# apirrone/Open_Duck_Playground

Measured on AMD Instinct MI355X. Metric: env-steps/sec open_duck_mini_v2 flat_terrain @8192 envs; 1/2/4/8-GPU scaling, higher is better.
Workload: dtype f32

## Files before the change

include/odk.h:

```cpp
#ifndef ODK_H
#define ODK_H

#include <stdint.h>

#ifdef __cplusplus
extern "C" {
#endif

typedef struct odk_model odk_model;
typedef struct odk_batch odk_batch;

enum odk_status {
  ODK_OK = 0,
  ODK_ERR_INVALID = -1,
  ODK_ERR_UNSUPPORTED = -2,
  ODK_ERR_HIP = -3,
  ODK_ERR_NOMEM = -4
};

#define ODK_NOBS 101
#define ODK_NPRIV 212
#define ODK_NOBS_STANDING 85
#define ODK_NPRIV_STANDING 153
#define ODK_ENV_JOYSTICK 0
#define ODK_ENV_STANDING 1
#define ODK_NMETRIC 8
#define ODK_NU 14

typedef struct {
  float ctrl_dt, action_scale, dof_vel_scale, max_motor_velocity;
  float noise_level, noise_gyro, noise_accelerometer, noise_gravity, noise_joint_vel;
  float qpos_noise_scale[16];
  float reward_scales[7];
  float tracking_sigma;
  float push_enable, push_interval_range[2], push_magnitude_range[2];
  float cmd_range[7][2];
  int32_t use_imitation, use_motor_speed_limits;
  int32_t autoreset;
  int32_t episode_length;
  int32_t n_substeps;
  int32_t lanes_per_env;
  int32_t env_kind;
  float reset_base_qvel;
  int32_t hfield_up_normals_only;
} odk_env_config;

typedef struct {
  float* obs_dev;
  float* priv_dev;
  float* reward_dev;
  float* done_dev;
  float* truncation_dev;
  float* metrics_dev;
} odk_outputs;

enum odk_param {
  ODK_PARAM_BODY_MASS = 0,
  ODK_PARAM_BODY_IPOS_TORSO = 1,
  ODK_PARAM_DOF_FRICTIONLOSS = 2,
  ODK_PARAM_DOF_ARMATURE = 3,
  ODK_PARAM_QPOS0 = 4,
  ODK_PARAM_KP = 5
};

const char* odk_last_error(void);
void odk_default_config(odk_env_config* cfg);
void odk_default_config_standing(odk_env_config* cfg);
void odk_obs_sizes(int env_kind, int* nobs, int* npriv);

int odk_model_load(const void* blob, uint64_t len, odk_model** out);
void odk_model_free(odk_model* m);
int odk_model_dims(const odk_model* m, int* nq, int* nv, int* nu, int* nbody);
int odk_model_obs_sizes(const odk_model* m, int env_kind, int* nobs, int* npriv);

int odk_model_reduced(const odk_model* m, int* paired, int* nvr, int* nMr, int* nHr, int* red_main, int* red_twin);
int odk_model_body_lanes(const odk_model* m, int lanes_per_env, int* out, int n);
int odk_model_env_lds_floats(const odk_model* m);

int odk_batch_create(const odk_model* m, const odk_env_config* cfg, int nenv, int device, const float* prm_table,
                     const double* dxs, int nx, const double* dys, int ny, const double* dths, int nth, const double* ranges6,
                     int nsteps_in_period, odk_batch** out);
void odk_batch_destroy(odk_batch* b);
int odk_batch_set_config(odk_batch* b, const odk_env_config* cfg);

int odk_batch_set_param(odk_batch* b, int param, const float* host_values, int count_per_env);

int odk_reset(odk_batch* b, uint32_t seed, uint32_t env_id_offset, const odk_outputs* outs, void* stream);

int odk_step(odk_batch* b, const float* action_dev, const odk_outputs* outs, void* stream);

int odk_batch_bind_commands(odk_batch* b, const float* cmd_dev, int row_stride);

#define ODK_NXTERM 12
enum odk_xterm {
  ODK_XTERM_LIN_VEL_Z = 0, ODK_XTERM_ANG_VEL_XY = 1, ODK_XTERM_ORIENTATION = 2, ODK_XTERM_BASE_HEIGHT = 3, ODK_XTERM_ENERGY = 4,
  ODK_XTERM_JOINT_POS_LIMITS = 5, ODK_XTERM_TERMINATION = 6, ODK_XTERM_POSE = 7, ODK_XTERM_FEET_SLIP = 8, ODK_XTERM_FEET_CLEARANCE = 9,
  ODK_XTERM_FEET_HEIGHT = 10, ODK_XTERM_FEET_AIR_TIME = 11
};
typedef struct {
  float scale[ODK_NXTERM];
  float base_height_target;
  float max_foot_height;
  float air_time_range[2];
  float soft_joint_pos_limit_factor;
  float pose_weight[16];
} odk_reward_terms;
int odk_batch_set_reward_terms(odk_batch* b, const odk_reward_terms* terms);
int odk_batch_bind_reward_metrics(odk_batch* b, float* dev);

int odk_batch_set_imitation_joints(odk_batch* b, const int32_t* frame_joint, int nu);

int odk_batch_set_head_joints(odk_batch* b, const int32_t* actuator, int n);

#define ODK_TRACK_NACC 12
enum { ODK_TRACK_ENDED = 0, ODK_TRACK_STEPS = 1, ODK_TRACK_SAMPLES = 2, ODK_TRACK_FALLS = 3, ODK_TRACK_REWARD = 4, ODK_TRACK_SUM = 5,
       ODK_TRACK_SQERR = 8 };
int odk_tracking_accumulate(const odk_batch* b, const float* priv_dev, const float* reward_dev, const float* done_dev,
                            const float* truncation_dev, float* acc_dev, void* stream);

int odk_batch_bind_pushes(odk_batch* b, const float* push_dev, int row_stride);

int odk_batch_bind_action_delays(odk_batch* b, const int32_t* delay_dev, int row_stride);

#define ODK_PUSH_NACC 10
enum { ODK_PUSH_PUSHED = 0, ODK_PUSH_PUSH_AT = 1, ODK_PUSH_FELL = 2, ODK_PUSH_STEPS_TO_FALL = 3, ODK_PUSH_LAST_OFF = 4, ODK_PUSH_PEAK_LIN_ERR = 5,
       ODK_PUSH_PEAK_ANG_ERR = 6, ODK_PUSH_PRE_LIN_ERR_SUM = 7, ODK_PUSH_PRE_SAMPLES = 8, ODK_PUSH_PRE_LIN_ERR_LOW = 9 };
int odk_push_accumulate(const odk_batch* b, const float* priv_dev, const float* done_dev, const float* truncation_dev,
                        const float* track_acc_dev, float lin_tol, float ang_tol, float* acc_dev, void* stream);

#define ODK_GAIT_NACC 144
#define ODK_GAIT_STRIDE 16
enum { ODK_GAIT_SAMPLES = 0, ODK_GAIT_SPEED_SUM = 1, ODK_GAIT_ABS_POWER_SUM = 2, ODK_GAIT_CONTACT = 3, ODK_GAIT_DOUBLE = 5, ODK_GAIT_FLIGHT = 6,
       ODK_GAIT_TOUCHDOWNS = 7, ODK_GAIT_SWING_STEPS_SUM = 9, ODK_GAIT_SLIP_SUM = 11, ODK_GAIT_HEIGHT_SUM = 13, ODK_GAIT_HEIGHT_SQ_SUM = 14,
       ODK_GAIT_ROLLPITCH_RATE_SQ_SUM = 15, ODK_GAIT_ACTION_RATE_SUM = 16, ODK_GAIT_PREV_CONTACT = 17, ODK_GAIT_AIR_RUN = 19,
       ODK_GAIT_TORQUE_SQ = 32, ODK_GAIT_TORQUE_PEAK = 48, ODK_GAIT_VEL_PEAK = 64, ODK_GAIT_SAT = 80, ODK_GAIT_ABS_POWER = 96,
       ODK_GAIT_RANGE_MIN = 112, ODK_GAIT_RANGE_MAX = 128 };
int odk_gait_accumulate(const odk_batch* b, const float* priv_dev, const float* done_dev, const float* truncation_dev,
                        const float* track_acc_dev, const float* torque_limit_dev , float* acc_dev ,
                        void* stream);

#define ODK_POSTURE_NACC 32
enum { ODK_POSTURE_SAMPLES = 0, ODK_POSTURE_DRIFT_SPEED_SUM = 1, ODK_POSTURE_YAW_RATE_SQ_SUM = 2, ODK_POSTURE_ROLLPITCH_RATE_SQ_SUM = 3,
       ODK_POSTURE_TILT_SUM = 4, ODK_POSTURE_TILT_PEAK = 5, ODK_POSTURE_HEIGHT_SUM = 6, ODK_POSTURE_LEG_POSE_SUM = 7, ODK_POSTURE_LEG_VEL_SUM = 8,
       ODK_POSTURE_HEAD_SQERR_SUM = 9, ODK_POSTURE_ANGLE_SUM = 16, ODK_POSTURE_ERR_SQ_SUM = 20, ODK_POSTURE_ERR_PEAK = 24,
       ODK_POSTURE_LAST_OFF = 28 };
int odk_posture_accumulate(const odk_batch* b, const float* priv_dev, const float* done_dev, const float* truncation_dev,
                           const float* track_acc_dev, float tol, float* acc_dev , void* stream);

#define ODK_IMIT_NACC 160
#define ODK_IMIT_STRIDE 16
enum { ODK_IMIT_SAMPLES = 0, ODK_IMIT_GATED = 1, ODK_IMIT_SPEED_ERR_SQ_SUM = 2, ODK_IMIT_REF_SPEED_SUM = 3, ODK_IMIT_JOINT_POS_SQ_SUM = 4,
       ODK_IMIT_JOINT_VEL_SQ_SUM = 5, ODK_IMIT_BOTH = 6, ODK_IMIT_ROBOT_ONLY = 8, ODK_IMIT_REF_ONLY = 10, ODK_IMIT_REF_TOUCHDOWNS = 12,
       ODK_IMIT_TOUCHDOWNS = 14, ODK_IMIT_LAG_SUM = 16, ODK_IMIT_LAG_ABS_SUM = 18, ODK_IMIT_PREV_CONTACT = 20, ODK_IMIT_PREV_REF = 22,
       ODK_IMIT_REF_AGE = 24,
       ODK_IMIT_POS_ERR_SUM = 32, ODK_IMIT_POS_ERR_SQ = 48, ODK_IMIT_POS_ERR_PEAK = 64, ODK_IMIT_VEL_ERR_SQ = 80, ODK_IMIT_RANGE_MIN = 96,
       ODK_IMIT_RANGE_MAX = 112, ODK_IMIT_REF_RANGE_MIN = 128, ODK_IMIT_REF_RANGE_MAX = 144 };
int odk_imitation_accumulate(const odk_batch* b, const float* priv_dev, const float* done_dev, const float* truncation_dev,
                             const float* track_acc_dev, int period_steps, float* acc_dev , void* stream);

#define ODK_SCHED_MAX_SEGMENTS 8
// ... 158 lines not shown
```

open_duck_playground_amd/csrc/odk_env_kernels.h:

```cpp
#pragma once
#include <hip/hip_runtime.h>

#include "odk_shapes.h"
#include "odk_poison.h"



template <class S> __device__ __forceinline__ const int* load_shared(float* lds, int envs, const DevModel* m) {
  int* RT = reinterpret_cast<int*>(lds + envs * EnvL<S>::TOTAL);
  {
    constexpr int T = (S::NMR + 63) / 64;
    int v[T];
#pragma unroll
    for (int t = 0; t < T; t++) { const int k = threadIdx.x + 64 * t; v[t] = m->R_ent[k < S::NMR ? k : 0]; }
#pragma unroll
    for (int t = 0; t < T; t++) { const int k = threadIdx.x + 64 * t; if (k < S::NMR) RT[k] = v[t]; }
  }
  float* SH = reinterpret_cast<float*>(RT);
  float* CT = SH + S::SH_CT;
  const int k = threadIdx.x;
  if (k < 3) { CT[k] = m->pair_mu[k]; CT[3 + k] = m->pair_invweight[k]; }
  if (k < 27) CT[6 + k] = m->pair_imp[k / 9][k % 9];
  if (k < 9) CT[33 + k] = m->plane_frame[k];
  return RT;
}

__device__ __forceinline__ float i2f(int v) { return __int_as_float(v); }
__device__ __forceinline__ int f2i(float v) { return __float_as_int(v); }
__device__ __forceinline__ float nan_to_num(float x) {
  if (isnan(x)) return 0.0f;
  if (isinf(x)) return x > 0 ? 3.4028234663852886e38f : -3.4028234663852886e38f;
  return x;
}

template <class S, int G>
__device__ __noinline__ void dump_lds(float* dbg, const float* L, int env, int lane) {
  float* o = dbg + (size_t)env * S::TOTAL;
#pragma unroll 1
  for (int k = lane; k < S::TOTAL; k += G) o[k] = L[k];
}

template <int N, int G> struct G2L {
  static constexpr int T = (N + G - 1) / G;
  float v[T];
  __device__ __forceinline__ void load(const float* __restrict__ src, int lane) {
#pragma unroll
    for (int t = 0; t < T; t++) { const int i = lane + t * G; v[t] = src[i < N ? i : 0]; }
  }
  __device__ __forceinline__ void store(float* dst, int lane) const {
#pragma unroll
    for (int t = 0; t < T; t++) { const int i = lane + t * G; if (i < N) dst[i] = v[t]; }
  }
};

template <class S, int G>
struct ParamLoad {
  float q0, mass, arm, frl, kp, ipos, dq0, darm, dfrl;
  int qadr, dadr;
  __device__ __forceinline__ void load(const DevModel* __restrict__ m, const float* __restrict__ dr, int lane) {
    static_assert(S::NQ <= G && S::NV <= G && S::NB <= G && S::NU <= G, "one parameter of each kind per lane");
    const int iq = lane < S::NQ ? lane : 0, ib = lane < S::NB ? lane : 0, iv = lane < S::NV ? lane : 0, iu = lane < S::NU ? lane : 0, i3 = lane < 3 ? lane : 0;
    q0 = m->qpos0[iq];
    mass = dr ? dr[DRL<S>::MASS + ib] : m->body_mass[ib];
    arm = m->dof_armature[iv]; frl = m->dof_frictionloss[iv];
    kp = dr ? dr[DRL<S>::KP + iu] : m->act_kp[iu];
    ipos = dr ? dr[DRL<S>::IPOS + i3] : m->body_ipos[1][i3];
    qadr = m->act_qposadr[iu]; dadr = m->act_dofadr[iu];
    dq0 = dr ? dr[DRL<S>::Q0 + iu] : 0.0f; darm = dr ? dr[DRL<S>::ARM + iu] : 0.0f; dfrl = dr ? dr[DRL<S>::FRL + iu] : 0.0f;
  }
  __device__ __forceinline__ void store(float* L, bool has_dr, int lane) const {
    if (lane < S::NQ) L[S::O_Q0 + lane] = q0;
    if (lane < S::NB) L[S::O_MASS + lane] = mass;
    if (lane < S::NV) { L[S::O_ARM + lane] = arm; L[S::O_FRL + lane] = frl; }
    if (lane < S::NU) L[S::O_KP + lane] = kp;
    if (lane < 3) L[S::O_IPOS1 + lane] = ipos;
    ODK_SYNC();
    if (has_dr && lane < S::NU) { L[S::O_Q0 + qadr] = dq0; L[S::O_ARM + dadr] = darm; L[S::O_FRL + dadr] = dfrl; }
    ODK_SYNC();
  }
};
template <class S, int G>
__device__ __forceinline__ void load_params(float* L, const DevModel* m, const float* dr, int lane) {
  ParamLoad<S, G> p;
  p.load(m, dr, lane);
  p.store(L, dr != nullptr, lane);
}

__device__ __forceinline__ int prm_nearest(const float* grid, int n, float v) {
  int best = 0;
  float bd = fabsf(grid[0] - v);
#pragma unroll
  for (int i = 1; i < 16; i++) { const float d = fabsf(grid[i] - v); if (i < n && d < bd) { bd = d; best = i; } }
  return best;
}
template <int G>
__device__ __forceinline__ void prm_eval(const DevPRM* __restrict__ p, const float* table, float dx, float dy, float dth, int i, float* out, int lane) {
  const float x = fminf(fmaxf(dx, p->ranges[0]), p->ranges[1]);
  const float y = fminf(fmaxf(dy, p->ranges[2]), p->ranges[3]);
  const float t3 = fminf(fmaxf(dth, p->ranges[4]), p->ranges[5]);
  const int ix = prm_nearest(p->dxs, p->nx, x), iy = prm_nearest(p->dys, p->ny, y), it = prm_nearest(p->dths, p->nth, t3);
  float t = (float)(i % p->nsteps) / (float)p->nsteps;
  t = fminf(fmaxf(t, 0.0f), 1.0f);
  const float* c = table + ((size_t)((ix * p->ny + iy) * p->nth + it)) * 640;
  for (int k = lane; k < 40; k += G) {
    float yv = c[k * 16];
#pragma unroll
// ... 200 lines not shown
  if (lane == 2) {
    const float yaw = -3.14f + rng_uniform(k0, kr, 0, 2) * 6.28f;
    float s, co;
    sincosf(0.5f * yaw, &s, &co);
    float q0[4] = {L[S::O_QPOS + 3], L[S::O_QPOS + 4], L[S::O_QPOS + 5], L[S::O_QPOS + 6]}, qz[4] = {co, 0, 0, s}, r[4];
    qmul(r, q0, qz);
    for (int k = 0; k < 4; k++) L[S::O_QPOS + 3 + k] = r[k];
  }
  if (lane >= 3 && lane < 9) L[S::O_QVEL + lane - 3] = -c.reset_base_qvel + rng_uniform(k0, kr, 0, 3 + NU + lane - 3) * (2.0f * c.reset_base_qvel);
  for (int u = lane; u < S::NU; u += G) {
    const float v = L[S::O_QPOS + m->act_qposadr[u]] * (0.5f + rng_uniform(k0, kr, 0, 3 + u));
    L[S::O_QPOS + m->act_qposadr[u]] = v;
    L[S::O_CTRL + u] = v;
    INFO[RL.MT + u] = c.kind != 0 ? 0.0f : m->key_ctrl[u];
  }
  if (lane < 7) {
    float v;
    sample_command(c, k0, kr, 0, 9 + NU, lane, v);
    if (a.cmd) v = a.cmd[(size_t)e * a.cmd_stride + lane];
    INFO[RL.CMD + lane] = v;
  }
  ODK_SYNC();
  forward_env<S, G, HF>(L, RT, m, a.hfield, st, lane, 1);
  if (a.dbg_lds && live) dump_lds<S, G>(a.dbg_lds, L, env, lane);
  const float pint = c.push_interval_range[0] + rng_uniform(k0, kr, 0, 17 + NU) * (c.push_interval_range[1] - c.push_interval_range[0]);
  const int push_interval_steps = (int)rintf(pint / c.ctrl_dt);
  if (c.use_imitation) prm_eval<G>(&a.prm, a.prm_table, INFO[RL.CMD], INFO[RL.CMD + 1], INFO[RL.CMD + 2], 0, L + E::O_REF, lane);
  else for (int k = lane; k < 40; k += G) L[E::O_REF + k] = 0;
  ODK_SYNC();
  float contact[2];
  foot_contact_flags(L + S::O_CDIST, contact);
  const float phase[2] = {0, 0};
  draw_block<E::NDRAW>(k0, k1, 0u, L + E::O_NZ, lane);
  build_obs<S, G>(L, m, c, contact, L + E::O_NZ, 0, phase, c.noise_level != 0.0f, lane);
  if (lane == 0) {
    INFO[RL.KEY0] = i2f((int)k0); INFO[RL.KEY1] = i2f((int)k1); INFO[RL.CTR] = i2f(1);
    INFO[RL.STEP] = i2f(0); INFO[RL.PSTEP] = i2f(0); INFO[RL.PINT] = i2f(push_interval_steps);
    INFO[RL.IMI] = i2f(0); INFO[RL.LCON] = i2f(0);
  }
  ODK_SYNC();
  if (live) {
    float* rc = a.recs + (size_t)env * R::SIZE;
    float* fs = a.first + (size_t)env * R::FSIZE;
    for (int i = lane; i < S::NQ; i += G) { rc[i] = L[S::O_QPOS + i]; fs[i] = L[S::O_QPOS + i]; }
    for (int i = lane; i < S::NV; i += G) {
      rc[S::NQ + i] = L[S::O_QVEL + i]; fs[S::NQ + i] = L[S::O_QVEL + i];
      rc[S::NQ + S::NV + i] = L[S::O_WARM + i]; fs[S::NQ + S::NV + i] = L[S::O_WARM + i];
    }
    for (int k = lane; k < R::NPRIV; k += G) {
      if (k < R::NOBS) fs[R::FOBS + k] = L[E::O_PRIV + k];
      fs[R::FOBS + R::NOBS + k] = L[E::O_PRIV + k];
    }
    for (int k = lane; k < RL.NINFO; k += G) rc[R::INFO + k] = INFO[k];
    float metrics[ODK_NMETRIC] = {0, 0, 0, 0, 0, 0, 0, 0};
    write_outputs<S, G>(a, L, env, 0.0f, 0.0f, 0.0f, metrics, lane);
    if (a.xmet && lane < ODK_NXTERM) a.xmet[(size_t)env * ODK_NXTERM + lane] = 0.0f;
  }
}

constexpr int STEP_WAVES = 2;
#ifdef ODK_PROFILE
constexpr bool STEP_DUMPS_ALWAYS = true;
#else
constexpr bool STEP_DUMPS_ALWAYS = false;
#endif
template <class S, int G, int HF, bool DBG>
__device__ __forceinline__ void step_body(const KArgs& a) {
  extern __shared__ float lds[];
  using E = EnvL<S>; using R = Rec<S>;
  constexpr int NU = S::NU;
  constexpr RecLay RL = rec_lay(NU);
  const int slot = threadIdx.x / G, lane = threadIdx.x % G;
  const int env = blockIdx.x * (64 / G) + slot;
  const bool live = env < a.nenv;
  const int e = live ? env : a.nenv - 1;
  float* L = lds + slot * E::TOTAL;
#ifdef ODK_PROFILE
  const long long t_k0 = clock64();
#endif
#ifdef ODK_POISON_LDS
  odk_poison_fill(lds, E::wg_floats(64 / G));
  ODK_SYNC();
#endif
  const int* RT = load_shared<S>(lds, 64 / G, a.m);
  const DevModel* m = a.m;
  const EnvCfg& c = a.cfg;
  float* INFO = L + E::O_INFO; float* ACT = L + E::O_ACT; float* CTRL = L + S::O_CTRL;
  float* rc = a.recs + (size_t)e * R::SIZE;
  {
    G2L<S::NQ + 2 * S::NV, G> g_state;
    G2L<RL.NINFO, G> g_info;
    G2L<NU, G> g_act;
    ParamLoad<S, G> g_par;
    const float* drp = a.dr ? a.dr + (size_t)e * DRL<S>::SIZE : nullptr;
    g_state.load(rc, lane); g_info.load(rc + R::INFO, lane); g_act.load(a.action + (size_t)e * NU, lane);
    g_par.load(m, drp, lane);
    g_state.store(L + S::O_QPOS, lane); g_info.store(INFO, lane); g_act.store(ACT, lane);
    g_par.store(L, drp != nullptr, lane);
  }
  if (a.cmd) {
    if (lane < 7) INFO[RL.CMD + lane] = a.cmd[(size_t)e * a.cmd_stride + lane];
    ODK_SYNC();
  }
#ifdef ODK_PROFILE
  for (int k = lane; k < 36; k += G) L[S::O_SCR + S::S_PROF + k] = 0;
#endif
  Statics<S, G> st;
  load_statics<S, G>(st, m, lane);
  const uint32_t k0 = (uint32_t)f2i(INFO[RL.KEY0]), k1 = (uint32_t)f2i(INFO[RL.KEY1]), ctr = (uint32_t)f2i(INFO[RL.CTR]);
  int step = f2i(INFO[RL.STEP]), push_step = f2i(INFO[RL.PSTEP]);
  const int push_int = f2i(INFO[RL.PINT]);
  int imi = f2i(INFO[RL.IMI]);
  const int lcon = f2i(INFO[RL.LCON]);
  const float prev_done = INFO[RL.DONE];
  float ep_steps = prev_done != 0.0f ? 0.0f : INFO[RL.EPSTEPS];
  const float dt = c.ctrl_dt;
  float phase[2] = {0, 0};
  float ref0 = 0.0f, ref1 = 0.0f;
  if (c.use_imitation) {
    imi = (imi + 1) % a.prm.nsteps;
    const float ph = ((float)imi / (float)a.prm.nsteps) * 2.0f * PI_F;
    phase[0] = cosf(ph); phase[1] = sinf(ph);
    prm_eval_regs<G>(&a.prm, a.prm_table, INFO[RL.CMD], INFO[RL.CMD + 1], INFO[RL.CMD + 2], imi, ref0, ref1, lane);
  } else {
    imi = 0;
  }
  float h0 = 0, h1 = 0;
  for (int u = lane; u < NU; u += G) { h0 = INFO[RL.AHIST + u]; h1 = INFO[RL.AHIST + NU + u]; }
  ODK_SYNC();
  for (int u = lane; u < NU; u += G) { INFO[RL.AHIST + u] = ACT[u]; INFO[RL.AHIST + NU + u] = h0; INFO[RL.AHIST + 2 * NU + u] = h1; }
  ODK_SYNC();
  uint32_t w0, w1, w2, w3;
  threefry2x32(k0, k1, ctr, 0u, w0, w1);
  threefry2x32(k0, k1, ctr, 1u, w2, w3);
  int aidx = randint3((float)(w0 >> 8) * (1.0f / 16777216.0f));
  const float theta = (float)(w2 >> 8) * (1.0f / 16777216.0f) * (2.0f * PI_F);
  const float mag = c.push_magnitude_range[0] + (float)(w3 >> 8) * (1.0f / 16777216.0f) * (c.push_magnitude_range[1] - c.push_magnitude_range[0]);
  const float gate = (((push_step + 1) % push_int) == 0 ? 1.0f : 0.0f) * c.push_enable;
  float push[2] = {cosf(theta) * gate, sinf(theta) * gate};
  if (a.push) {
    if (lane < 2) {
      const float* pr = a.push + (size_t)e * a.push_stride;
      const float kx = pr[0], ky = pr[1];
      L[S::O_QVEL + lane] += lane == 0 ? kx : ky;
      const float n2 = kx * kx + ky * ky;
      const float inv = n2 > 0.0f ? 1.0f / sqrtf(n2) : 0.0f;
      push[0] = kx * inv; push[1] = ky * inv;
    }
  } else if (lane < 2) {
    L[S::O_QVEL + lane] += push[lane] * mag;
  }
  if (lane == 0) {
    INFO[RL.PUSH] = push[0]; INFO[RL.PUSH + 1] = push[1];
    INFO[RL.IMI] = i2f(imi);
    ACT[NU] = phase[0]; ACT[NU + 1] = phase[1];
    INFO[RL.EPSTEPS] = ep_steps;
  }
  if (a.delay) {
    const int d = a.delay[(size_t)e * a.delay_stride];
    if (d >= 0) aidx = d < 2 ? d : 2;
  }
  for (int u = lane; u < NU; u += G) {
    float mt = m->key_ctrl[u] + INFO[RL.AHIST + aidx * NU + u] * c.action_scale;
    if (c.use_motor_speed_limits) {
      const float prev = INFO[RL.MT + u], lim = c.max_motor_velocity * dt;
      mt = fminf(fmaxf(mt, prev - lim), prev + lim);
    }
// ... 232 lines not shown
```

open_duck_playground_amd/csrc/odk_kernels.h:

```cpp
#pragma once
#include <hip/hip_runtime.h>

#include "odk_model.h"

namespace odk {

#define ODK_SYNC() asm volatile("" ::: "memory")

constexpr float MINVAL_F = 1e-15f;
constexpr float PI_F = 3.14159265358979323846f;

struct EnvCfg {
  float ctrl_dt, action_scale, dof_vel_scale, max_motor_velocity;
  float noise_level, noise_gyro, noise_accelerometer, noise_gravity, noise_joint_vel;
  float qpos_noise_scale[16];
  float reward_scales[7];
  float tracking_sigma;
  float push_enable, push_interval_range[2], push_magnitude_range[2];
  float cmd_range[7][2];
  int use_imitation, use_motor_speed_limits, autoreset, episode_length, n_substeps;
  int kind, nobs, npriv;
  float reset_base_qvel;
};

template <int NQ_, int NV_, int NB_, int NU_, int NJ_, int NM_, int NH_, int NROW_, int DT_, int DV_, bool CONE_ = false, int CL_ = -1, bool OPT_ = false, int NCH_ = 3>
struct Shape {
  static constexpr int NQ = NQ_, NV = NV_, NB = NB_, NU = NU_, NJ = NJ_, NM = NM_, NH = NH_, NROW = NROW_;
  static constexpr int DT = DT_;
  static constexpr int DV = DV_;
  static constexpr int NCROW = 48;
  static constexpr bool PAIRED = (NV_ == 30);
  static constexpr int MAXJB = PAIRED ? 2 : 1;
  static constexpr bool EQ = (NV_ == 21) || OPT_;
  static constexpr bool CONE = CONE_;
  static constexpr bool ELL = (NV_ == 21) || CONE_ || OPT_;
  static constexpr int NVR = PAIRED ? 20 : NV_;
  static constexpr int NMR = PAIRED ? 145 : NM_;
  static constexpr int NHR = PAIRED ? 170 : NH_;
  static constexpr int DVR = PAIRED ? 15 : DV_;
  static constexpr int SH_CT = NMR, SHARED = SH_CT + 42;
  static constexpr int CL = CL_ >= 0 ? CL_ : ((NV_ == 20 || NV_ == 21 || PAIRED) ? 5 : 0);
  static constexpr int NCH = NCH_;
  static_assert(NCH >= 1 && NCH <= 4, "chain_solve: one 8-lane group per chain, 32 lanes");
  static constexpr int O_QPOS = 0;
  static constexpr int O_QVEL = O_QPOS + NQ;
  static constexpr int O_WARM = O_QVEL + NV;
  static constexpr int O_CTRL = O_WARM + NV;
  static constexpr int O_Q0 = O_CTRL + NU;
  static constexpr int O_MASS = O_Q0 + NQ;
  static constexpr int O_ARM = O_MASS + NB;
  static constexpr int O_FRL = O_ARM + NV;
  static constexpr int O_KP = O_FRL + NV;
  static constexpr int O_IPOS1 = O_KP + NU;
  static constexpr int O_XPOS = O_IPOS1 + 3;
  static constexpr int O_XQUAT = O_XPOS + 3 * NB;
  static constexpr int O_CVEL = O_XQUAT + 4 * NB;
  static constexpr int O_CACC = O_CVEL + 6 * NB;
  static constexpr int O_CFRC = O_CACC + 6 * NB;
  static constexpr int O_CRB = O_CFRC + 6 * NB;
  static constexpr int O_CDOF = O_CRB + 10 * NB;
  static constexpr int O_BUF6 = O_CDOF + 6 * NVR;
  static constexpr int O_BUF6B = O_BUF6 + 6 * NVR;
  static constexpr int O_M = O_BUF6B + 6 * NVR;
  static constexpr int O_HL = O_M + NMR;
  static constexpr int O_QFS = O_HL + NHR;
  static constexpr int O_QAS = O_QFS + NV;
  static constexpr int O_X = O_QAS + NV;
  static constexpr int O_MA = O_X + NV;
  static constexpr int O_GRAD = O_MA + NV;
  static constexpr int O_MV = O_GRAD + NV;
  static constexpr int O_D = O_MV + NV;
  static constexpr int O_AREF = O_D + NROW;
  static constexpr int O_JAR = O_AREF + NROW;
  static constexpr int O_JV = O_JAR + NROW;
  static constexpr int O_SC = O_JAR;
  static_assert(2 * NJ <= NROW, "sin/cos must fit in the jar rows");
  static constexpr bool W_FITS = 6 * NCROW <= 16 * NB;
  static constexpr int O_CDIST = O_JV + NROW;
  static constexpr int O_CR = O_CDIST + NCON;
  static constexpr int O_SCR = O_CR + 3 * NCON;
  static constexpr int S_VF = 0;
  static constexpr int S_FF = 12;
  static constexpr int S_K = 24;
  static constexpr int S_FR = S_K;
  static constexpr int S_VF2 = 132;
  static constexpr int S_FFX = 144;
  static constexpr int S_EQ = 150;
  static constexpr int S_SOLVE_END = S_K + 7 * NCH * CL + 27;
  static constexpr int S_MISC = S_SOLVE_END > 156 ? S_SOLVE_END : 156;
  static constexpr int S_PROF = S_MISC + 16;
  static constexpr int S_PROF2 = S_PROF + 20;
#ifdef ODK_PROFILE
  static constexpr int N_SCR = S_PROF2 + 16;
#else
  static constexpr int N_SCR = ((S_MISC + 16 + 3) / 4) * 4;
#endif
  static constexpr int O_SENS = O_JV;
  static_assert(NSENSD <= NROW, "sensordata must fit in the jv rows");
  static constexpr int O_ACTF = O_SCR + N_SCR;
  static constexpr int O_QACC = O_X;
  static constexpr int O_EQP = ((O_ACTF + NU + 3) / 4) * 4;
  static constexpr int EQP_W = 0, EQP_J = 12 * EQP_ROWS, EQP_D = EQP_J + EQP_ROWS * NV, EQP_AREF = EQP_D + EQP_ROWS, EQP_POS = EQP_AREF + EQP_ROWS;
  static constexpr int N_EQP = EQ ? ((EQP_POS + EQP_ROWS + 3) / 4) * 4 : 0;
  static constexpr int O_WX = O_EQP + N_EQP;
  static constexpr int O_W = W_FITS ? O_CFRC : O_WX;
  static constexpr int TOTAL = O_WX + (W_FITS ? 0 : 6 * NCROW);
  static constexpr int N_INFO = ((43 + 7 * NU + 3) / 4) * 4, N_ACT = ((NU + 2 + 3) / 4) * 4;
  static constexpr int ENV_STRIDE = TOTAL + N_INFO + N_ACT;
};

#ifdef ODK_PROFILE
#define ODK_PROF(i) do { if (lane == 0) { long long _t = clock64(); SCR[S::S_PROF + (i)] += (float)(_t - _tprev); _tprev = _t; } } while (0)
#define ODK_PROF_BEGIN() long long _tprev = clock64()
#elif defined(ODK_MARK)
#define ODK_PROF(i) asm volatile("; ODK_PHASE_END " #i ::: "memory")
#define ODK_PROF_BEGIN() asm volatile("; ODK_PHASE_BEGIN" ::: "memory")
#else
#define ODK_PROF(i) do { } while (0)
#define ODK_PROF_BEGIN() do { } while (0)
#endif

#define ODK_DPP(v, ctrl, rmask) __int_as_float(__builtin_amdgcn_update_dpp(0, __float_as_int(v), ctrl, rmask, 0xF, true))
struct OpSum { static __device__ __forceinline__ float f(float a, float b) { return a + b; } };
struct OpMax { static __device__ __forceinline__ float f(float a, float b) { return fmaxf(a, b); } };
struct OpMin { static __device__ __forceinline__ float f(float a, float b) { return fminf(a, b); } };
typedef unsigned int odk_u2 __attribute__((ext_vector_type(2)));
template <int G, class Op> __device__ __forceinline__ float greduce(float v) {
  v = Op::f(v, ODK_DPP(v, 0xB1, 0xF));
  v = Op::f(v, ODK_DPP(v, 0x4E, 0xF));
  v = Op::f(v, ODK_DPP(v, 0x141, 0xF));
  v = Op::f(v, ODK_DPP(v, 0x140, 0xF));
  const unsigned iv = __float_as_uint(v);
  const odk_u2 h = __builtin_amdgcn_permlane16_swap(iv, iv, false, false);
  v = Op::f(__uint_as_float(h[0]), __uint_as_float(h[1]));
  if (G == 64) {
    const unsigned iw = __float_as_uint(v);
    const odk_u2 w = __builtin_amdgcn_permlane32_swap(iw, iw, false, false);
    v = Op::f(__uint_as_float(w[0]), __uint_as_float(w[1]));
  }
  return v;
}
template <int G> __device__ __forceinline__ float gsum(float v) { return greduce<G, OpSum>(v); }
__device__ __forceinline__ float row_shr(float v, int si) { return si == 0 ? ODK_DPP(v, 0x111, 0xF) : si == 1 ? ODK_DPP(v, 0x112, 0xF) : ODK_DPP(v, 0x114, 0xF); }
__device__ __forceinline__ float row_shl(float v, int si) { return si == 0 ? ODK_DPP(v, 0x101, 0xF) : si == 1 ? ODK_DPP(v, 0x102, 0xF) : ODK_DPP(v, 0x104, 0xF); }
template <int G, int N> __device__ __forceinline__ void gsum_n(float* v) {
  if constexpr (G == 32) {
    float o[N];
#pragma unroll
    for (int i = 0; i < N; i++) {
      float x = v[i];
      x += ODK_DPP(x, 0xB1, 0xF); x += ODK_DPP(x, 0x4E, 0xF); x += ODK_DPP(x, 0x141, 0xF); x += ODK_DPP(x, 0x140, 0xF);
      v[i] = x;
      o[i] = __int_as_float(__builtin_amdgcn_ds_swizzle(__float_as_int(x), 0x401F));
    }
#pragma unroll
    for (int i = 0; i < N; i++) v[i] += o[i];
  } else {
#pragma unroll
    for (int i = 0; i < N; i++) v[i] = gsum<G>(v[i]);
  }
}
__device__ __forceinline__ unsigned fkey(float v) { const unsigned b = __float_as_uint(v); return b ^ ((b >> 31) ? 0xFFFFFFFFu : 0x80000000u); }
__device__ __forceinline__ float fkey_inv(unsigned k) { return __uint_as_float(k ^ ((k >> 31) ? 0x80000000u : 0xFFFFFFFFu)); }
#define ODK_DPPU(v, ctrl) ((unsigned)__builtin_amdgcn_update_dpp(0, (int)(v), ctrl, 0xF, 0xF, true))
template <int G, bool MAX> __device__ __forceinline__ unsigned greduce_u(unsigned v) {
  auto op = [](unsigned a, unsigned b) { return MAX ? (a > b ? a : b) : (a < b ? a : b); };
  v = op(v, ODK_DPPU(v, 0xB1));
  v = op(v, ODK_DPPU(v, 0x4E));
  v = op(v, ODK_DPPU(v, 0x141));
  v = op(v, ODK_DPPU(v, 0x140));
  const odk_u2 h = __builtin_amdgcn_permlane16_swap(v, v, false, false);
  v = op(h[0], h[1]);
  if (G == 64) {
    const odk_u2 w = __builtin_amdgcn_permlane32_swap(v, v, false, false);
    v = op(w[0], w[1]);
  }
  return v;
}
template <int G> __device__ __forceinline__ float gmax(float v) { return fkey_inv(greduce_u<G, true>(fkey(v))); }
template <int G> __device__ __forceinline__ float gmin(float v) { return fkey_inv(greduce_u<G, false>(fkey(v))); }
template <int G> __device__ __forceinline__ int gargmax(float v, int i) {
  const unsigned k = fkey(v);
  const unsigned mx = greduce_u<G, true>(k);
  return (int)greduce_u<G, false>(k == mx ? (unsigned)i : 0x7FFFFFFFu);
}
template <int G> __device__ __forceinline__ float bcast(float v, int j) {
  const int iv = __float_as_int(v);
  if (G == 64) return __int_as_float(__builtin_amdgcn_readlane(iv, j));
  const int lo = __builtin_amdgcn_readlane(iv, j), hi = __builtin_amdgcn_readlane(iv, j + 32);
  return __int_as_float((threadIdx.x & 32) ? hi : lo);
}
__device__ __forceinline__ int ubcast(int v, int j) { return __builtin_amdgcn_readlane(v, j); }

__device__ __forceinline__ void cross3(float* r, const float* a, const float* b) {
  float x = a[1] * b[2] - a[2] * b[1], y = a[2] * b[0] - a[0] * b[2], z = a[0] * b[1] - a[1] * b[0];
  r[0] = x; r[1] = y; r[2] = z;
}
__device__ __forceinline__ float dot3(const float* a, const float* b) { return a[0] * b[0] + a[1] * b[1] + a[2] * b[2]; }
__device__ __forceinline__ void qmul(float* r, const float* a, const float* b) {
  float w = a[0] * b[0] - a[1] * b[1] - a[2] * b[2] - a[3] * b[3];
  float x = a[0] * b[1] + a[1] * b[0] + a[2] * b[3] - a[3] * b[2];
  float y = a[0] * b[2] - a[1] * b[3] + a[2] * b[0] + a[3] * b[1];
  float z = a[0] * b[3] + a[1] * b[2] - a[2] * b[1] + a[3] * b[0];
  r[0] = w; r[1] = x; r[2] = y; r[3] = z;
}
__device__ __forceinline__ void qnormalize(float* q) {
  const float n2 = q[0] * q[0] + q[1] * q[1] + q[2] * q[2] + q[3] * q[3];
  if (n2 < MINVAL_F * MINVAL_F) { q[0] = 1; q[1] = q[2] = q[3] = 0; return; }
  const float inv = __builtin_amdgcn_rsqf(n2);
  q[0] *= inv; q[1] *= inv; q[2] *= inv; q[3] *= inv;
}
__device__ __forceinline__ void qrot(float* r, const float* q, const float* v) {
  float t[3], u[3] = {q[1], q[2], q[3]}, c[3];
  cross3(t, u, v);
  t[0] *= 2; t[1] *= 2; t[2] *= 2;
  cross3(c, u, t);
  r[0] = v[0] + q[0] * t[0] + c[0]; r[1] = v[1] + q[0] * t[1] + c[1]; r[2] = v[2] + q[0] * t[2] + c[2];
}
__device__ __forceinline__ void q2mat(float* m, const float* q) {
  float w = q[0], x = q[1], y = q[2], z = q[3];
  m[0] = w * w + x * x - y * y - z * z; m[1] = 2 * (x * y - w * z); m[2] = 2 * (x * z + w * y);
  m[3] = 2 * (x * y + w * z); m[4] = w * w - x * x + y * y - z * z; m[5] = 2 * (y * z - w * x);
  m[6] = 2 * (x * z - w * y); m[7] = 2 * (y * z + w * x); m[8] = w * w - x * x - y * y + z * z;
}
__device__ __forceinline__ void inert_mul(float* res, const float* i, const float* v) {
  res[0] = i[0] * v[0] + i[3] * v[1] + i[4] * v[2] - i[8] * v[4] + i[7] * v[5];
  res[1] = i[3] * v[0] + i[1] * v[1] + i[5] * v[2] + i[8] * v[3] - i[6] * v[5];
  res[2] = i[4] * v[0] + i[5] * v[1] + i[2] * v[2] - i[7] * v[3] + i[6] * v[4];
  res[3] = i[8] * v[1] - i[7] * v[2] + i[9] * v[3];
  res[4] = i[6] * v[2] - i[8] * v[0] + i[9] * v[4];
  res[5] = i[7] * v[0] - i[6] * v[1] + i[9] * v[5];
}
__device__ __forceinline__ void cross_motion(float* res, const float* vel, const float* v) {
  float a[3], b[3];
  cross3(res, vel, v);
  cross3(a, vel, v + 3);
  cross3(b, vel + 3, v);
  res[3] = a[0] + b[0]; res[4] = a[1] + b[1]; res[5] = a[2] + b[2];
}

__device__ __forceinline__ uint32_t rotl32(uint32_t x, int r) { return (x << r) | (x >> (32 - r)); }
__device__ inline void threefry2x32(uint32_t k0, uint32_t k1, uint32_t c0, uint32_t c1, uint32_t& o0, uint32_t& o1) {
  const int R[8] = {13, 15, 26, 6, 17, 29, 16, 24};
  uint32_t ks[3] = {k0, k1, 0x1BD11BDAu ^ k0 ^ k1};
  uint32_t x0 = c0 + ks[0], x1 = c1 + ks[1];
#pragma unroll
  for (int blk = 0; blk < 5; blk++) {
#pragma unroll
    for (int r = 0; r < 4; r++) {
      x0 += x1;
      x1 = rotl32(x1, R[(blk & 1) * 4 + r]);
      x1 ^= x0;
    }
    x0 += ks[(blk + 1) % 3];
    x1 += ks[(blk + 2) % 3] + (uint32_t)(blk + 1);
  }
  o0 = x0; o1 = x1;
}
__device__ inline float rng_uniform(uint32_t k0, uint32_t k1, uint32_t ctr, uint32_t idx) {
  uint32_t a, b;
  threefry2x32(k0, k1, ctr, idx >> 1, a, b);
  return (float)(((idx & 1) ? b : a) >> 8) * (1.0f / 16777216.0f);
}
__device__ __forceinline__ int randint3(float u) { int i = (int)(u * 3.0f); return i > 2 ? 2 : i; }

template <class S, int G>
struct Statics : LaneSt {
  static constexpr int NME = (S::NMR + G - 1) / G;
  static constexpr int NHE = (S::NHR + G - 1) / G;
  static_assert((S::NVR + 1) / 2 <= 16, "LaneSt::m_adr");
};
struct ActSt { float bias2, clo, chi, flo, fhi; int climited, flimited; };
struct FlSt { float D, R, b; int dof; };

struct HotSt { ActSt as; FlSt fs; float vb[3]; };

template <class S, int G>
__device__ __forceinline__ void load_statics(Statics<S, G>& st, const DevModel* __restrict__ m, int lane) {
  static_cast<LaneSt&>(st) = m->lane_st[lane];
}
template <class S>
__host__ __device__ inline void compute_statics(LaneSt& st, const DevModel* m, int lane) {
  {
    const bool on = lane >= 1 && lane < S::NJ;
    st.j_qadr = on ? m->jnt_qposadr[on ? lane : 0] : -1;
    st.j_dadr = m->jnt_dofadr[on ? lane : 0];
  }
  {
    st.cs_pk = 0;
    const int c = lane >> 3;
    if (c < S::NCH && c < m->nrchain) {
      const int f = m->rchain_first[c];
      st.cs_pk = m->rchain_len[c] | (m->red_depth[f] << 3) | (f << 8) | (m->red_Madr[f] << 14);
    }
    int tb = 0, tb2 = 0;
    if (lane < 21) { while ((tb + 1) * (tb + 2) / 2 <= lane) tb++; tb2 = lane - tb * (tb + 1) / 2; }
    else if (lane < 27) { tb = lane - 21; tb2 = 6; }
    st.cs_pk |= (tb << 24) | (tb2 << 27);
  }
  st.ch_first = 0; st.ch_len = 0;
  for (int c = 0; c < 4; c++)
    if (c < m->nrchain && lane >= m->rchain_first[c] && lane < m->rchain_first[c] + m->rchain_len[c]) { st.ch_first = m->rchain_first[c]; st.ch_len = m->rchain_len[c]; }
  {
    const int r = lane < S::NVR ? lane : 0;
    st.r_on = lane < S::NVR;
    st.r_depth = m->red_depth[r]; st.r_Madr = m->red_Madr[r]; st.r_ancmask = m->red_ancmask[r]; st.r_descmask = m->red_descmask[r];
    st.r_foot = st.r_on ? m->red_foot[r] : 0;
    if (!st.r_on) { st.r_ancmask = 0; st.r_descmask = 0; st.r_depth = 0; }
    const int rel = st.r_ancmask | st.r_descmask | (st.r_on ? (1 << r) : 0);
    for (int jp = 0; jp < (S::NVR + 1) / 2; jp++) {
      int pk = 0;
      for (int h = 0; h < 2; h++) {
        const int j = 2 * jp + h;
        int off = S::O_CDOF * 4;
        if (j < S::NVR && ((rel >> j) & 1)) off = (S::O_M + (j < r ? st.r_Madr + m->red_depth[j] : m->red_Madr[j] + st.r_depth)) * 4;
        pk |= off << (16 * h);
      }
      st.m_adr[jp] = pk;
    }
  }
  const int i = lane < S::NV ? lane : 0;
  st.d_on = lane < S::NV;
  st.d_body = m->dof_body[i];
  st.d_act = st.d_on ? m->dof_act[i] : -1;
  st.d_flrow = st.d_on ? m->dof_flrow[i] : -1;
  st.d_limrow = st.d_on ? m->dof_limrow[i] : -1;
  st.d_foot = st.d_on ? (m->foot_dofmask[0][i] | (m->foot_dofmask[1][i] << 1)) : 0;
  st.d_damping = m->dof_damping[i];
  st.d_lim_on = st.d_limrow >= 0;
  st.d_qadr = m->dof_qadr[i];
  st.d_lo = m->dof_range[i][0]; st.d_hi = m->dof_range[i][1];
  st.d_tkind = (S::PAIRED && st.d_on) ? m->dof_tkind[i] : 0;
  st.d_red = S::PAIRED ? m->dof_red[i] : i;
}
template <int G>
__device__ __forceinline__ void load_body(BodySt& b, const DevModel* __restrict__ m, int lane) {
  b = m->body_st[G == 64][lane];
}
__device__ __forceinline__ void load_act(ActSt& a, const DevModel* __restrict__ m, int act) {
  const int u = act >= 0 ? act : 0;
  a.bias2 = m->act_bias2[u]; a.clo = m->act_ctrlrange[u][0]; a.chi = m->act_ctrlrange[u][1];
  a.flo = m->act_forcerange[u][0]; a.fhi = m->act_forcerange[u][1];
  a.climited = m->act_ctrllimited[u]; a.flimited = m->act_forcelimited[u];
}
__device__ __forceinline__ void load_fl(FlSt& f, const DevModel* __restrict__ m, int lane) {
  const int r = lane < m->nfl ? lane : 0;
  f.D = m->fl_D[r]; f.R = m->fl_R[r]; f.b = m->fl_b[r]; f.dof = m->fl_dof[r];
}
template <class S, int G>
__device__ __forceinline__ void load_hot(HotSt& h, const DevModel* __restrict__ m, const Statics<S, G>& st, int lane) {
  load_act(h.as, m, st.d_act);
  load_fl(h.fs, m, lane);
  const int f = (lane >> 4) & 1, j = lane & 15;
  const int jv = (lane < 32 && j < m->foot_nvert[f]) ? j : 0;
  for (int k = 0; k < 3; k++) h.vb[k] = m->foot_vert[f][jv][k];
}
__device__ __forceinline__ int load_rent(const DevModel* __restrict__ m, int p, int n) { const int e = m->R_ent[p < n ? p : 0]; return p < n ? e : -1; }
__device__ __forceinline__ int load_rhent(const DevModel* __restrict__ m, int p, int n) { const int e = m->RH_ent[p < n ? p : 0]; return p < n ? e : -1; }

template <int G, int DMAX, int NVT>
__device__ __forceinline__ void factor_rows(float* A, int lane, int on, int di, int ai, int descmask, int depth_st, int madr_st) {
  float row[DMAX > 0 ? DMAX : 1];
#pragma unroll
  for (int c = 0; c < DMAX; c++) row[c] = A[ai + c];
  float diag = A[ai + di];
  if (!on) diag = 1.0f;
  for (int k = NVT - 1; k > 0; k--) {
    const int Dk = ubcast(depth_st, k);
    if (Dk == 0) continue;
    const int ak = ubcast(madr_st, k);
    if (lane == k) {
      const float inv = __builtin_amdgcn_rcpf(diag);
#pragma unroll
      for (int c = 0; c < DMAX; c++)
        if (c < Dk) { row[c] *= inv; A[ak + c] = row[c]; }
      A[ak + Dk] = diag;
    }
    ODK_SYNC();
    {
      const bool anc = (descmask >> k) & 1;
      float rk[DMAX > 0 ? DMAX : 1];
#pragma unroll
      for (int c = 0; c < DMAX; c++) rk[c] = A[ak + c];
      const float Lki = A[ak + di], dk = A[ak + Dk];
      const float t = anc ? Lki * dk : 0.0f;
#pragma unroll
      for (int c = 0; c < DMAX; c++) row[c] = anc ? fmaf(-t, rk[c], row[c]) : row[c];
      diag = anc ? fmaf(-t, Lki, diag) : diag;
    }
    ODK_SYNC();
  }
  if (on) A[ai + di] = diag;
  ODK_SYNC();
}

template <int G, int DMAX, int NVT, int MAXLEN, int NBASE>
__device__ __forceinline__ void factor_chains(float* A, int lane, int on, int di, int ai, int ch_first, int ch_len, int descmask,
                                              int depth_st, int madr_st) {
  float row[DMAX > 0 ? DMAX : 1];
#pragma unroll
  for (int c = 0; c < DMAX; c++) row[c] = A[ai + c];
  float diag = A[ai + di];
  if (!on) diag = 1.0f;
  const int a_loc = lane - ch_first;
#pragma unroll
  for (int s = 0; s < MAXLEN; s++) {
    const int kl = ch_len - 1 - s;
    const int t = kl - a_loc;
    const bool act = ch_len > 0 && kl >= 0;
    if (act && t == 0) {
      const float inv = __builtin_amdgcn_rcpf(diag);
#pragma unroll
      for (int c = 0; c < DMAX; c++)
        if (c < DMAX - s && c < di) { row[c] *= inv; A[ai + c] = row[c]; }
      A[ai + di] = diag;
    }
    ODK_SYNC();
    {
      const bool anc = act && t > 0;
      const int tk = anc ? t : 0;
      const int ak = ai + tk * (di + 1) + (tk * (tk - 1)) / 2, Dk = di + tk;
      float rk[DMAX > 0 ? DMAX : 1];
#pragma unroll
      for (int c = 0; c < DMAX; c++)
        if (c < DMAX - s - 1) rk[c] = A[ak + c];
      const float Lki = A[ak + di], dk = A[ak + Dk];
      const float tt = anc ? Lki * dk : 0.0f;
#pragma unroll
      for (int c = 0; c < DMAX; c++)
        if (c < DMAX - s - 1) row[c] = anc ? fmaf(-tt, rk[c], row[c]) : row[c];
      diag = anc ? fmaf(-tt, Lki, diag) : diag;
    }
    ODK_SYNC();
  }
  {
    const bool chain = on && ch_len > 0;
    float mine = 0.0f;
    int q = 0;
#pragma unroll
// ... 1108 lines not shown
    for (int t = 0; t < 3; t++) { wp[t] = row_get(bp[0][t], src); wn[t] = row_get(bn[0][t], src); }
    const bool any = wi != 0x7FFFFFFFu && k < ncon;
    if (j == 0) {
      const int c = 4 * f + k;
      float pw[3], nw[3];
      for (int a = 0; a < 3; a++) {
        pw[a] = ph[a] + Rh[3 * a] * (wp[0] + org[0]) + Rh[3 * a + 1] * (wp[1] + org[1]) + Rh[3 * a + 2] * wp[2];
        nw[a] = any ? Rh[3 * a] * wn[0] + Rh[3 * a + 1] * wn[1] + Rh[3 * a + 2] * wn[2] : Rh[3 * a + 2];
      }
      CDIST[c] = any ? vm : 1.0f;
      for (int t = 0; t < 3; t++) CR[3 * c + t] = any ? pw[t] - ref[t] : 0.0f;
      make_frame_dev(nw, FR + 9 * c);
    }
    if (mine) {
      bd[0] = bd[1]; bidx[0] = bidx[1]; bd[1] = 3.0e38f; bidx[1] = 0x7FFFFFFF;
      for (int t = 0; t < 3; t++) { bp[0][t] = bp[1][t]; bn[0][t] = bn[1][t]; }
    }
  }
  if (j < 2) {
    const int c = 4 * f + 2 + j;
    const float up[3] = {Rh[2], Rh[5], Rh[8]};
    CDIST[c] = 1.0f; CR[3 * c] = 0.0f; CR[3 * c + 1] = 0.0f; CR[3 * c + 2] = 0.0f;
    make_frame_dev(up, FR + 9 * c);
  }
}

struct ConeEv { float N, T, U1, U2, Dm, NmT; int zone; };
__device__ __forceinline__ float cone_dm(float Dn, float mur) { return Dn * __builtin_amdgcn_rcpf(fmaxf(mur * mur * (1.0f + mur * mur), MINVAL_F)); }
__device__ __forceinline__ ConeEv cone_ev(float Dn, float Dm, float mu, float mur, float xn, float x1, float x2) {
  ConeEv e;
  e.U1 = mu * x1; e.U2 = mu * x2; e.N = mur * xn;
  e.T = __builtin_amdgcn_sqrtf(e.U1 * e.U1 + e.U2 * e.U2);
  e.Dm = Dm;
  e.NmT = e.N - mur * e.T;
  const bool top = (e.N >= mur * e.T) || (e.T <= 0.0f && e.N >= 0.0f) || !(Dn > 0.0f);
  const bool bot = (mur * e.N + e.T <= 0.0f) || (e.T <= 0.0f && e.N < 0.0f);
  e.zone = top ? 0 : (bot ? 1 : 2);
  return e;
}
__device__ __forceinline__ float cone_cost(const ConeEv& e, float Dn, float Dt, float xn, float x1, float x2) {
  return e.zone == 0 ? 0.0f : (e.zone == 1 ? 0.5f * (Dn * xn * xn + Dt * (x1 * x1 + x2 * x2)) : 0.5f * e.Dm * e.NmT * e.NmT);
}
__device__ __forceinline__ float cone_force(const ConeEv& e, float Dn, float Dt, float mu, float mur, float xn, float x1, float x2, int s) {
  if (e.zone == 0 || s > 2) return 0.0f;
  if (e.zone == 1) return s == 0 ? -Dn * xn : -Dt * (s == 1 ? x1 : x2);
  const float fn = -e.Dm * e.NmT * mur;
  return s == 0 ? fn : -fn * __builtin_amdgcn_rcpf(e.T) * (s == 1 ? e.U1 : e.U2) * mu;
}
__device__ __forceinline__ void cone_hess_row(const ConeEv& e, float Dn, float Dt, float mu, float mur, int s, float* C) {
  C[0] = C[1] = C[2] = 0.0f;
  if (e.zone == 0 || s > 2) return;
  if (e.zone == 1) { C[s] = s == 0 ? Dn : Dt; return; }
  const float iT = __builtin_amdgcn_rcpf(e.T);
  const float g[3] = {1.0f, -mur * e.U1 * iT, -mur * e.U2 * iT}, Sc[3] = {mur, mu, mu};
  const float i3 = iT * iT * iT, p11 = e.U2 * e.U2 * i3, p12 = -e.U1 * e.U2 * i3, p22 = e.U1 * e.U1 * i3;
  const float P[3] = {0.0f, s == 1 ? p11 : (s == 2 ? p12 : 0.0f), s == 1 ? p12 : (s == 2 ? p22 : 0.0f)};
  const float gs = s == 0 ? g[0] : (s == 1 ? g[1] : g[2]), Ss = s == 0 ? mur : mu;
#pragma unroll
  for (int b = 0; b < 3; b++) {
    const float h = e.Dm * gs * g[b] - e.Dm * e.NmT * mur * P[b];
    C[b] = Ss * h * Sc[b];
  }
}
__device__ __forceinline__ void cone_line(float Dn, float Dt, float Dm, float mu, float mur, const float* x, const float* v, float& cost, float& d0, float& d1) {
  const ConeEv e = cone_ev(Dn, Dm, mu, mur, x[0], x[1], x[2]);
  const float c1 = 0.5f * (Dn * x[0] * x[0] + Dt * (x[1] * x[1] + x[2] * x[2]));
  const float a1 = Dn * x[0] * v[0] + Dt * (x[1] * v[1] + x[2] * v[2]);
  const float b1 = Dn * v[0] * v[0] + Dt * (v[1] * v[1] + v[2] * v[2]);
  const float V0 = v[0] * mur, V1 = v[1] * mu, V2 = v[2] * mu;
  const float UV = e.U1 * V1 + e.U2 * V2, iT = __builtin_amdgcn_rcpf(e.zone == 2 ? e.T : 1.0f);
  const float cr = e.U1 * V2 - e.U2 * V1;
  const float T1 = UV * iT, T2 = cr * cr * iT * iT * iT;
  const float g1 = V0 - mur * T1;
  const float c2 = 0.5f * e.Dm * e.NmT * e.NmT, a2 = e.Dm * e.NmT * g1, b2 = e.Dm * (g1 * g1 - e.NmT * mur * T2);
  cost = e.zone == 0 ? 0.0f : (e.zone == 1 ? c1 : c2);
  d0 = e.zone == 0 ? 0.0f : (e.zone == 1 ? a1 : a2);
  d1 = e.zone == 0 ? 0.0f : (e.zone == 1 ? b1 : b2);
}

template <class S, int G, int HF, bool PRE = false, bool DBG = true>
__device__ __forceinline__ void forward_env(float* L, const int* RT, const DevModel* __restrict__ m, const float* __restrict__ hfield, const Statics<S, G>& st, int lane, int flags, const HotSt& hot = HotSt()) {
  const float* SH = reinterpret_cast<const float*>(RT);
  const float* CT = SH + S::SH_CT;
  constexpr int NV = S::NV, NB = S::NB, NR = S::NVR;
  using ST = Statics<S, G>;
  float* QPOS = L + S::O_QPOS; float* QVEL = L + S::O_QVEL; float* WARM = L + S::O_WARM; float* CTRL = L + S::O_CTRL;
  float* Q0 = L + S::O_Q0; float* MASS = L + S::O_MASS; float* ARM = L + S::O_ARM; float* FRL = L + S::O_FRL; float* KP = L + S::O_KP;
  float* XPOS = L + S::O_XPOS; float* XQUAT = L + S::O_XQUAT; float* CVEL = L + S::O_CVEL; float* CACC = L + S::O_CACC;
  float* CFRC = L + S::O_CFRC; float* CRB = L + S::O_CRB; float* SC = L + S::O_SC; float* CDOF = L + S::O_CDOF;
  float* BUF6 = L + S::O_BUF6; float* BUF6B = L + S::O_BUF6B; float* M = L + S::O_M; float* HL = L + S::O_HL;
  float* QFS = L + S::O_QFS; float* QAS = L + S::O_QAS; float* X = L + S::O_X; float* MA = L + S::O_MA; float* GRAD = L + S::O_GRAD;
  float* MV = L + S::O_MV; float* ED = L + S::O_D; float* AREF = L + S::O_AREF; float* JAR = L + S::O_JAR; float* JV = L + S::O_JV;
  float* W = L + S::O_W; float* CDIST = L + S::O_CDIST; float* CR = L + S::O_CR; float* SCR = L + S::O_SCR;
  float* SENS = L + S::O_SENS; float* ACTF = L + S::O_ACTF;
  const int nfl = m->nfl, nlim = m->nlim, r0c = nfl + nlim;
  const float dt = m->dt;
  const float ref[3] = {QPOS[0], QPOS[1], QPOS[2]};
  ODK_PROF_BEGIN();

  BodySt bs;
  load_body<G>(bs, m, lane);
  const int bid = bs.body;
  if (st.j_qadr >= 0) {
    float s, c;
    const float x = 0.5f * (QPOS[st.j_qadr] - Q0[st.j_qadr]);
    if (fabsf(x) <= 1.7f) {
      const float x2 = x * x;
      float ps = 1.6059043836821613e-10f, pc = -1.1470745597729725e-11f;
      ps = fmaf(ps, x2, -2.505210838544172e-08f); pc = fmaf(pc, x2, 2.08767569878681e-09f);
      ps = fmaf(ps, x2, 2.7557319223985893e-06f); pc = fmaf(pc, x2, -2.755731922398589e-07f);
      ps = fmaf(ps, x2, -0.0001984126984126984f); pc = fmaf(pc, x2, 2.48015873015873e-05f);
      ps = fmaf(ps, x2, 0.008333333333333333f); pc = fmaf(pc, x2, -0.001388888888888889f);
      ps = fmaf(ps, x2, -0.16666666666666666f); pc = fmaf(pc, x2, 0.041666666666666664f);
      ps = fmaf(ps, x2, 1.0f); pc = fmaf(pc, x2, -0.5f);
      s = ps * x; c = fmaf(pc, x2, 1.0f);
    } else {
      sincosf(x, &s, &c);
    }
    SC[2 * lane] = s; SC[2 * lane + 1] = c;
  }
  ODK_SYNC();
  ODK_PROF(0);
  {
    float p[3], q[4], cvel[6] = {0, 0, 0, 0, 0, 0}, cacc[6] = {0, 0, 0, 0, 0, 0};
    {
      const bool stat = bs.level == -1;
      for (int k = 0; k < 3; k++) p[k] = stat ? bs.pos[k] : 0.0f;
      for (int k = 0; k < 4; k++) q[k] = stat ? bs.quat[k] : (k == 0 ? 1.0f : 0.0f);
    }
    const int max_np = m->max_nonpath_level;
    for (int lvl = 0; lvl <= max_np; lvl++) {
      if (bs.level == lvl && !bs.is_path) {
        if (lvl == 0) {
          for (int k = 0; k < 3; k++) p[k] = ref[k];
          for (int k = 0; k < 4; k++) q[k] = QPOS[3 + k];
          qnormalize(q);
          float R[9];
          q2mat(R, q);
          const float wl[3] = {QVEL[3], QVEL[4], QVEL[5]};
          float ww[3];
          for (int k = 0; k < 3; k++) ww[k] = R[3 * k] * wl[0] + R[3 * k + 1] * wl[1] + R[3 * k + 2] * wl[2];
          const float v[3] = {QVEL[0], QVEL[1], QVEL[2]};
          for (int k = 0; k < 3; k++) {
            for (int c = 0; c < 6; c++) CDOF[c * NR + k] = (c == 3 + k) ? 1.0f : 0.0f;
            CDOF[0 * NR + 3 + k] = R[k]; CDOF[1 * NR + 3 + k] = R[3 + k]; CDOF[2 * NR + 3 + k] = R[6 + k];
            CDOF[3 * NR + 3 + k] = 0; CDOF[4 * NR + 3 + k] = 0; CDOF[5 * NR + 3 + k] = 0;
          }
          float vxw[3];
          cross3(vxw, v, ww);
          cvel[0] = ww[0]; cvel[1] = ww[1]; cvel[2] = ww[2]; cvel[3] = v[0]; cvel[4] = v[1]; cvel[5] = v[2];
          cacc[3] = -m->gravity[0] + vxw[0]; cacc[4] = -m->gravity[1] + vxw[1]; cacc[5] = -m->gravity[2] + vxw[2];
        } else {
          const int pb = bs.parent;
          float pp[3], pq[4], t[3];
          for (int k = 0; k < 3; k++) pp[k] = XPOS[k * NB + pb];
          for (int k = 0; k < 4; k++) pq[k] = XQUAT[k * NB + pb];
          for (int k = 0; k < 6; k++) { cvel[k] = CVEL[k * NB + pb]; cacc[k] = CACC[k * NB + pb]; }
          qrot(t, pq, bs.pos);
          p[0] = pp[0] + t[0]; p[1] = pp[1] + t[1]; p[2] = pp[2] + t[2];
          qmul(q, pq, bs.quat);
#pragma unroll
          for (int jj = 0; jj < S::MAXJB; jj++) {
            if (jj < bs.njnt) {
              float axw[3], cd[6], dot[6];
              qrot(axw, q, bs.ax[jj]);
              const float off[3] = {ref[0] - p[0], ref[1] - p[1], ref[2] - p[2]};
              cd[0] = axw[0]; cd[1] = axw[1]; cd[2] = axw[2];
              cross3(cd + 3, axw, off);
              const int d = bs.jd[jj], col = bs.jr[jj];
              if (col >= 0) {
#pragma unroll
                for (int k = 0; k < 6; k++) CDOF[k * NR + col] = cd[k];
              }
              const float qv = QVEL[d];
              cross_motion(dot, cvel, cd);
#pragma unroll
              for (int k = 0; k < 6; k++) { cacc[k] += dot[k] * qv; cvel[k] += cd[k] * qv; }
              const float s = SC[2 * bs.jj[jj]], c = SC[2 * bs.jj[jj] + 1];
              const float qj[4] = {c, s * bs.ax[jj][0], s * bs.ax[jj][1], s * bs.ax[jj][2]};
              qmul(q, q, qj);
            }
          }
          qnormalize(q);
        }
#pragma unroll
        for (int k = 0; k < 3; k++) XPOS[k * NB + bid] = p[k];
#pragma unroll
        for (int k = 0; k < 4; k++) XQUAT[k * NB + bid] = q[k];
#pragma unroll
        for (int k = 0; k < 6; k++) { CVEL[k * NB + bid] = cvel[k]; CACC[k * NB + bid] = cacc[k]; }
      }
      ODK_SYNC();
    }
    {
      const bool isp = bs.is_path != 0, head = bs.path_head != 0;
      float ql[4] = {bs.quat[0], bs.quat[1], bs.quat[2], bs.quat[3]}, qb[S::MAXJB][4];
#pragma unroll
      for (int jj = 0; jj < S::MAXJB; jj++) {
#pragma unroll
        for (int k = 0; k < 4; k++) qb[jj][k] = ql[k];
        if (jj < bs.njnt) {
          const float s = SC[2 * bs.jj[jj]], c = SC[2 * bs.jj[jj] + 1];
          const float qj[4] = {c, s * bs.ax[jj][0], s * bs.ax[jj][1], s * bs.ax[jj][2]};
          qmul(ql, ql, qj);
        }
      }
      float tp[3] = {bs.pos[0], bs.pos[1], bs.pos[2]}, tq[4] = {ql[0], ql[1], ql[2], ql[3]};
      float ppq[4] = {1, 0, 0, 0}, pcv[6] = {0, 0, 0, 0, 0, 0}, pca[6] = {0, 0, 0, 0, 0, 0};
      if (isp && head) {
        const int pb = bs.parent;
        float pp[3], t[3];
        for (int k = 0; k < 3; k++) pp[k] = XPOS[k * NB + pb];
        for (int k = 0; k < 4; k++) ppq[k] = XQUAT[k * NB + pb];
// ... 86 lines not shown
#pragma unroll
        for (int k = 0; k < 6; k++) ca[k] += row_shr(ok ? ca[k] : 0.0f, si);
      }
      if (isp) {
        qnormalize(tq);
#pragma unroll
        for (int k = 0; k < 3; k++) { p[k] = tp[k]; XPOS[k * NB + bid] = tp[k]; }
#pragma unroll
        for (int k = 0; k < 4; k++) { q[k] = tq[k]; XQUAT[k * NB + bid] = tq[k]; }
#pragma unroll
        for (int k = 0; k < 6; k++) { cvel[k] = cv[k]; cacc[k] = ca[k]; CVEL[k * NB + bid] = cv[k]; CACC[k * NB + bid] = ca[k]; }
      }
      ODK_SYNC();
    }
    float acc[16];
    if (bid >= 0 && bs.level < 0) {
#pragma unroll
      for (int k = 0; k < 3; k++) XPOS[k * NB + bid] = p[k];
#pragma unroll
      for (int k = 0; k < 4; k++) XQUAT[k * NB + bid] = q[k];
#pragma unroll
      for (int k = 0; k < 6; k++) { CVEL[k * NB + bid] = 0; CACC[k * NB + bid] = 0; }
    }
    {
      float R[9];
      q2mat(R, q);
      float ip[3] = {bs.ipos[0], bs.ipos[1], bs.ipos[2]};
      {
        const float i0 = L[S::O_IPOS1], i1 = L[S::O_IPOS1 + 1], i2 = L[S::O_IPOS1 + 2];
        asm volatile("" :: "v"(i0), "v"(i1), "v"(i2));
        ip[0] = bid == 1 ? i0 : ip[0]; ip[1] = bid == 1 ? i1 : ip[1]; ip[2] = bid == 1 ? i2 : ip[2];
      }
      float off[3];
      for (int k = 0; k < 3; k++) off[k] = p[k] + R[3 * k] * ip[0] + R[3 * k + 1] * ip[1] + R[3 * k + 2] * ip[2] - ref[k];
      const float* f = bs.inertia;
      const float Ib[9] = {f[0], f[3], f[4], f[3], f[1], f[5], f[4], f[5], f[2]};
      float T[9], Iw[9];
      for (int i = 0; i < 3; i++)
        for (int j = 0; j < 3; j++) T[3 * i + j] = R[3 * i] * Ib[j] + R[3 * i + 1] * Ib[3 + j] + R[3 * i + 2] * Ib[6 + j];
      for (int i = 0; i < 3; i++)
        for (int j = 0; j < 3; j++) Iw[3 * i + j] = T[3 * i] * R[3 * j] + T[3 * i + 1] * R[3 * j + 1] + T[3 * i + 2] * R[3 * j + 2];
      const float mb = MASS[bid >= 0 ? bid : 0], o2 = dot3(off, off);
      float ci[10];
      ci[0] = Iw[0] + mb * (o2 - off[0] * off[0]);
      ci[1] = Iw[4] + mb * (o2 - off[1] * off[1]);
      ci[2] = Iw[8] + mb * (o2 - off[2] * off[2]);
      ci[3] = Iw[1] - mb * off[0] * off[1];
      ci[4] = Iw[2] - mb * off[0] * off[2];
      ci[5] = Iw[5] - mb * off[1] * off[2];
      ci[6] = mb * off[0]; ci[7] = mb * off[1]; ci[8] = mb * off[2];
      ci[9] = mb;
      float fr[6], t1[6], a3[3], c3[3];
      inert_mul(fr, ci, cacc);
      inert_mul(t1, ci, cvel);
      cross3(a3, cvel, t1);
      cross3(c3, cvel + 3, t1 + 3);
      fr[0] += a3[0] + c3[0]; fr[1] += a3[1] + c3[1]; fr[2] += a3[2] + c3[2];
      cross3(a3, cvel, t1 + 3);
      fr[3] += a3[0]; fr[4] += a3[1]; fr[5] += a3[2];
      const bool dyn = bs.level >= 0;
#pragma unroll
      for (int k = 0; k < 10; k++) acc[k] = dyn ? ci[k] : 0.0f;
#pragma unroll
      for (int k = 0; k < 6; k++) acc[10 + k] = dyn ? fr[k] : 0.0f;
    }
    ODK_PROF(1);
#pragma unroll
    for (int si = 0; si < 3; si++) {
      const bool ok = (bs.upmask >> si) & 1;
#pragma unroll
      for (int k = 0; k < 16; k++) acc[k] += row_shl(ok ? acc[k] : 0.0f, si);
    }
    if (bid >= 0) {
#pragma unroll
      for (int k = 0; k < 10; k++) CRB[k * NB + bid] = acc[k];
#pragma unroll
      for (int k = 0; k < 6; k++) CFRC[k * NB + bid] = acc[10 + k];
    }
    ODK_SYNC();
  }
  {
    float* ACC = CFRC;
    static_assert(S::O_CRB == S::O_CFRC + 6 * NB, "cfrc | crb must be contiguous");
    const int nnp = m->np_count;
    const int slot = lane >> 4, q = lane & 15;
    float t[2] = {0.0f, 0.0f};
#pragma unroll
    for (int pass = 0; pass < 2; pass++) {
      const int i = pass * (G / 16) + slot;
      if (i < nnp) {
        const int ns = m->np_nsrc[i];
        int src[6];
#pragma unroll
        for (int c = 0; c < 6; c++) src[c] = m->np_src[i][c];
        float x = 0.0f;
#pragma unroll
        for (int c = 0; c < 6; c++) { const float y = ACC[q * NB + src[c]]; x += c < ns ? y : 0.0f; }
        t[pass] = x;
      }
    }
    ODK_SYNC();
#pragma unroll
    for (int pass = 0; pass < 2; pass++) {
      const int i = pass * (G / 16) + slot;
      if (i < nnp) ACC[q * NB + m->np_body[i]] = t[pass];
    }
    ODK_SYNC();
  }
  ODK_PROF(2);
  float qfs = 0.0f;
  if (st.d_on) {
    const int i = lane, b = st.d_body;
    float crb[10], cd[6], buf[6], bias = 0;
#pragma unroll
    for (int k = 0; k < 10; k++) crb[k] = CRB[k * NB + b];
#pragma unroll
    for (int k = 0; k < 6; k++) { cd[k] = CDOF[k * NR + st.d_red]; bias += cd[k] * CFRC[k * NB + b]; }
    inert_mul(buf, crb, cd);
    if (st.d_tkind != 2) {
#pragma unroll
      for (int k = 0; k < 6; k++) BUF6[k * NR + st.d_red] = buf[k];
    }
    const float qv = QVEL[i];
    float frc = -st.d_damping * qv - bias;
    const int u = st.d_act;
    if (u >= 0) {
      ActSt as;
      if constexpr (PRE) as = hot.as; else load_act(as, m, u);
      float ctrl = CTRL[u];
      if (as.climited) ctrl = fminf(fmaxf(ctrl, as.clo), as.chi);
      const float kp = KP[u];
      float af = kp * ctrl - kp * QPOS[st.d_qadr] + as.bias2 * qv;
      if (as.flimited) af = fminf(fmaxf(af, as.flo), as.fhi);
      ACTF[u] = af;
      frc += af;
    }
    QFS[i] = frc;
    qfs = frc;
  }
  ODK_SYNC();
  ODK_PROF(3);
  {
    int ee[ST::NME];
#pragma unroll
    for (int t = 0; t < ST::NME; t++) { const int pq = lane + t * G; ee[t] = RT[pq < S::NMR ? pq : 0]; }
    float vv[ST::NME];
#pragma unroll
    for (int t = 0; t < ST::NME; t++) {
      const int e = ee[t], i = e & 31, j = (e >> 5) & 31;
      const float arm = ARM[(e >> 16) & 31];
      float v = 0;
#pragma unroll
      for (int k = 0; k < 6; k++) v += CDOF[k * NR + j] * BUF6[k * NR + i];
      vv[t] = v + ((((e >> 14) & 3) == 1) ? arm : 0.0f);
    }
#pragma unroll
    for (int t = 0; t < ST::NME; t++) { const int pq = lane + t * G; if (pq < S::NMR) M[pq] = vv[t]; }
  }
  ODK_SYNC();
  ODK_PROF(4);
  float qas;
  if constexpr (S::PAIRED) {
    {
      int ee[ST::NME]; float mm[ST::NME];
#pragma unroll
      for (int t = 0; t < ST::NME; t++) { const int p = lane + t * G, pc = p < S::NMR ? p : 0; ee[t] = RT[pc]; mm[t] = M[pc]; }
#pragma unroll
      for (int t = 0; t < ST::NME; t++) {
        const float pe = pair_einv(ARM, nullptr, (ee[t] >> 16) & 31);
        mm[t] += ((ee[t] >> 15) & 1) ? pe : 0.0f;
      }
#pragma unroll
      for (int t = 0; t < ST::NME; t++) { const int p = lane + t * G; if (p < S::NMR) HL[p] = mm[t]; }
    }
    if (st.r_on) GRAD[lane] = pair_rhs<S>(QFS, ARM, nullptr, m, lane);
    ODK_SYNC();
    ODK_PROF(5);
    chain_solve<S, G>(HL, GRAD, SCR + S::S_K, BUF6, st.cs_pk, lane);
    qas = pair_expand<S, G>(GRAD, QFS, qfs, ARM, nullptr, st, lane);
    if (st.d_on) QAS[lane] = qas;
  } else if constexpr (S::CL > 0) {
    if (st.d_on) QAS[lane] = qfs;
    ODK_SYNC();
    chain_solve<S, G>(M, QAS, SCR + S::S_K, BUF6, st.cs_pk, lane);
    ODK_PROF(5);
    qas = st.d_on ? QAS[lane] : 0.0f;
  } else {
#pragma unroll
    for (int t = 0; t < ST::NME; t++) { const int p = lane + t * G; if (p < S::NMR) HL[p] = M[p]; }
    ODK_SYNC();
    if (m->nrchain > 0 && m->rchain_first[0] == 6)
      factor_chains<G, S::DT, NV, S::DT - 5, 6>(HL, lane, st.r_on, st.r_depth, st.r_Madr, st.ch_first, st.ch_len, st.r_descmask, st.r_depth, st.r_Madr);
    else
      factor_rows<G, S::DT, NV>(HL, lane, st.r_on, st.r_depth, st.r_Madr, st.r_descmask, st.r_depth, st.r_Madr);
    ODK_PROF(5);
    qas = solve_rows<G, NV>(HL, qfs, lane, st.r_on, st.r_depth, st.r_Madr, st.r_ancmask, st.r_descmask, st.r_depth, st.r_Madr);
    if (st.d_on) QAS[lane] = qas;
  }
  float mrow[NR];
  auto gather_M = [&]() {
    static_assert(S::CL > 0, "the zero entry of unrelated dofs is the floating base's CDOF[0][0]");
    static_assert(S::TOTAL * 4 < 65536, "16-bit byte offsets");
#pragma unroll
    for (int j = 0; j < NR; j++) {
      const unsigned off = ((unsigned)st.m_adr[j >> 1] >> (16 * (j & 1))) & 0xFFFFu;
      mrow[j] = *reinterpret_cast<const float*>(reinterpret_cast<const char*>(L) + off);
    }
  };
  auto mul_M = [&](const float* VB, float* YB, float vi) -> float {
    float acc0 = 0.0f, acc1 = 0.0f;
#pragma unroll
    for (int j = 0; j + 1 < NR; j += 2) { acc0 = fmaf(mrow[j], VB[j], acc0); acc1 = fmaf(mrow[j + 1], VB[j + 1], acc1); }
    if constexpr (NR & 1) acc0 = fmaf(mrow[NR - 1], VB[NR - 1], acc0);
    float acc = acc0 + acc1;
    if constexpr (S::PAIRED) {
      if (st.r_on) YB[lane] = acc;
      ODK_SYNC();
      acc = st.d_on ? YB[st.d_red] + (st.d_tkind != 0 ? ARM[lane] * vi : 0.0f) : 0.0f;
    }
    return acc;
  };
  ODK_SYNC();
  ODK_PROF(6);

  float fR[2][9], fP[2][3];
#pragma unroll
  for (int f = 0; f < 2; f++) {
    const int fb = m->foot_body[f];
    float q[4];
    for (int k = 0; k < 4; k++) q[k] = XQUAT[k * NB + fb];
    for (int k = 0; k < 3; k++) fP[f][k] = XPOS[k * NB + fb];
    q2mat(fR[f], q);
  }
  if constexpr (HF) {
    if constexpr (HF == 2) { hfield_prim_floor<S, G>(L, m, hfield, lane); ODK_SYNC(); prim_contacts<S, G>(L, m, lane, false); }
    else hfield_contacts<S, G>(L, m, hfield, lane);
  } else if (m->foot_prim) {
    prim_contacts<S, G>(L, m, lane, true);
  } else {
  const float pn0[3] = {m->plane_n[0], m->plane_n[1], m->plane_n[2]};
  {
    const int f = (lane >> 4) & 1, j = lane & 15;
    const int nvt = m->foot_nvert[f];
    const bool inrow = lane < 32;
    const bool has = inrow && j < nvt, has_e = inrow && nvt > 16;
    float pn[3] = {pn0[0], pn0[1], pn0[2]}, pp[3] = {m->plane_pos[0], m->plane_pos[1], m->plane_pos[2]};
    float Rf[9], Pf[3];
#pragma unroll
    for (int k = 0; k < 9; k++) Rf[k] = f ? fR[1][k] : fR[0][k];
#pragma unroll
    for (int k = 0; k < 3; k++) Pf[k] = f ? fP[1][k] : fP[0][k];
    float w[3] = {0, 0, 0}, we[3] = {0, 0, 0}, sup = -3.0e38f, supe = -3.0e38f;
    {
      const int jv = has ? j : 0;
      float vb[3];
      if constexpr (PRE) { vb[0] = hot.vb[0]; vb[1] = hot.vb[1]; vb[2] = hot.vb[2]; } else { vb[0] = m->foot_vert[f][jv][0]; vb[1] = m->foot_vert[f][jv][1]; vb[2] = m->foot_vert[f][jv][2]; }
      const float ve[3] = {m->foot_vert[f][16][0], m->foot_vert[f][16][1], m->foot_vert[f][16][2]};
#pragma unroll
      for (int k = 0; k < 3; k++) {
        w[k] = Pf[k] + Rf[3 * k] * vb[0] + Rf[3 * k + 1] * vb[1] + Rf[3 * k + 2] * vb[2];
        we[k] = Pf[k] + Rf[3 * k] * ve[0] + Rf[3 * k + 1] * ve[1] + Rf[3 * k + 2] * ve[2];
      }
      const float s0 = (pp[0] - w[0]) * pn[0] + (pp[1] - w[1]) * pn[1] + (pp[2] - w[2]) * pn[2];
      const float s1 = (pp[0] - we[0]) * pn[0] + (pp[1] - we[1]) * pn[1] + (pp[2] - we[2]) * pn[2];
      sup = has ? s0 : -3.0e38f; supe = has_e ? s1 : -3.0e38f;
    }
    int idx[4];
    select4_rows(w, has, sup, we, has_e, supe, nvt, pn, idx, lane);
#pragma unroll
    for (int k = 0; k < 4; k++) {
      bool uniq = true;
      for (int q = 0; q < k; q++) uniq = uniq && (idx[q] != idx[k]);
      const bool ext = idx[k] == 16;
      if (inrow && j == (ext ? 0 : idx[k])) {
        const float sv = ext ? supe : sup;
        const float dist = uniq ? -sv : 1.0f;
        const int c = 4 * f + k;
        CDIST[c] = dist;
        for (int t = 0; t < 3; t++) CR[3 * c + t] = (ext ? we[t] : w[t]) - 0.5f * dist * pn[t] - ref[t];
      }
    }
  }
  }
  ODK_PROF(7);
  if (!m->foot_prim) {
    float sep = -3.0e38f;
    float sph;
    {
      float dc[3];
      for (int k = 0; k < 3; k++) {
        const float a1 = fP[0][k] + fR[0][3 * k] * m->foot_obb_center[0][0] + fR[0][3 * k + 1] * m->foot_obb_center[0][1] + fR[0][3 * k + 2] * m->foot_obb_center[0][2];
        const float a2 = fP[1][k] + fR[1][3 * k] * m->foot_obb_center[1][0] + fR[1][3 * k + 1] * m->foot_obb_center[1][1] + fR[1][3 * k + 2] * m->foot_obb_center[1][2];
        dc[k] = a2 - a1;
      }
      sph = sqrtf(dot3(dc, dc)) - m->foot_sphere_r[0] - m->foot_sphere_r[1];
    }
    float boxsep = -3.0e38f;
    if (__builtin_amdgcn_ballot_w64(!(sph > 0.0f)) != 0) {
      if (lane < 15) {
        float c1[3], c2[3], A1[9], A2[9], tt[3];
  #pragma unroll
        for (int f = 0; f < 2; f++) {
          float* cc = f ? c2 : c1; float* AA = f ? A2 : A1;
          for (int k = 0; k < 3; k++) cc[k] = fP[f][k] + fR[f][3 * k] * m->foot_obb_center[f][0] + fR[f][3 * k + 1] * m->foot_obb_center[f][1] + fR[f][3 * k + 2] * m->foot_obb_center[f][2];
          for (int i = 0; i < 3; i++)
            for (int j = 0; j < 3; j++) AA[3 * i + j] = fR[f][3 * i] * m->foot_obb_axes[f][j] + fR[f][3 * i + 1] * m->foot_obb_axes[f][3 + j] + fR[f][3 * i + 2] * m->foot_obb_axes[f][6 + j];
        }
        for (int k = 0; k < 3; k++) tt[k] = c2[k] - c1[k];
        constexpr unsigned IA = 0u | 1u << 2 | 2u << 4 | 0u << 6 | 0u << 8 | 0u << 10 | 0u << 12 | 0u << 14 | 0u << 16 | 1u << 18 | 1u << 20 | 1u << 22 | 2u << 24 | 2u << 26 | 2u << 28;
        constexpr unsigned IB = 0u | 0u << 2 | 0u << 4 | 0u << 6 | 1u << 8 | 2u << 10 | 0u << 12 | 1u << 14 | 2u << 16 | 0u << 18 | 1u << 20 | 2u << 22 | 0u << 24 | 1u << 26 | 2u << 28;
        const int ia = (int)((IA >> (2 * lane)) & 3u), ib = (int)((IB >> (2 * lane)) & 3u);
        float e1[3], e2[3], ax[3];
  #pragma unroll
        for (int k = 0; k < 3; k++) {
          e1[k] = A1[3 * k + 2]; e1[k] = ia == 1 ? A1[3 * k + 1] : e1[k]; e1[k] = ia == 0 ? A1[3 * k] : e1[k];
          e2[k] = A2[3 * k + 2]; e2[k] = ib == 1 ? A2[3 * k + 1] : e2[k]; e2[k] = ib == 0 ? A2[3 * k] : e2[k];
        }
        cross3(ax, e1, e2);
        const float n = sqrtf(dot3(ax, ax));
        const bool edge = lane >= 6, ok = !edge | (n >= 1e-6f);
        const float inv = n >= 1e-6f ? 1.0f / n : 0.0f;
  #pragma unroll
        for (int k = 0; k < 3; k++) { ax[k] *= inv; ax[k] = lane < 6 ? e2[k] : ax[k]; ax[k] = lane < 3 ? e1[k] : ax[k]; }
        {
          float r1 = 0, r2 = 0;
  #pragma unroll
          for (int k = 0; k < 3; k++) {
            const float b1[3] = {A1[k], A1[3 + k], A1[6 + k]}, b2[3] = {A2[k], A2[3 + k], A2[6 + k]};
            r1 += m->foot_obb_half[0][k] * fabsf(dot3(ax, b1));
            r2 += m->foot_obb_half[1][k] * fabsf(dot3(ax, b2));
          }
          const float sv = fabsf(dot3(tt, ax)) - r1 - r2;
          sep = ok ? sv : sep;
        }
      }
      boxsep = gmax<G>(sep);
    }
    const float best = sph > 0.0f ? sph : boxsep;
    if (lane < 4) {
      const int c = 8 + lane;
      CDIST[c] = (lane == 0 && best > 0) ? best : 1.0f;
      CR[3 * c] = 0; CR[3 * c + 1] = 0; CR[3 * c + 2] = 0;
      if (lane == 0) SCR[S::S_MISC] = best;
    }
    const bool overlap = !(best > 0.0f);
    if (__builtin_amdgcn_ballot_w64(overlap) != 0) foot_foot_sat<S, G>(L, m, lane, overlap);
  }
  ODK_SYNC();
  ODK_PROF(8);

  FlSt fs;
  if constexpr (PRE) fs = hot.fs; else load_fl(fs, m, lane);
  float fl_f = 0.0f, fl_rf = 0.0f;
  if (lane < nfl) {
    fl_f = FRL[fs.dof]; fl_rf = fs.R * fl_f;
    ED[lane] = fs.D;
    AREF[lane] = -fs.b * QVEL[fs.dof];
  }
  float lim_sgn = 0.0f;
  if (st.d_lim_on) {
    const int r = nfl + st.d_limrow;
    const float qv = QPOS[st.d_qadr];
    const float dlo = qv - st.d_lo, dhi = st.d_hi - qv;
    const float pos = fminf(dlo, dhi);
    lim_sgn = dlo < dhi ? 1.0f : -1.0f;
    float D = 0, aref = 0;
    if (pos < 0) row_params(m->lim_imp[st.d_limrow], pos, m->lim_invweight[st.d_limrow], lim_sgn * QVEL[lane], D, aref);
    ED[r] = D; AREF[r] = aref;
  }
  bool eq_on = false, eq_first = false;
  int eq_i = 0, eq_j = -1, eq_r = 0;
  float eq_D = 0.0f, eq_aref = 0.0f, eq_c = 0.0f;
  if constexpr (S::EQ) {
    if (m->neq > 0 && st.d_on) {
      const int r = m->dof_eqrow[lane];
      if (r >= 0) {
        eq_on = true; eq_r = r; eq_i = m->eq_dof1[r]; eq_j = m->eq_dof2[r]; eq_first = lane == eq_i;
        const int a1 = m->eq_qadr1[r];
        const float* pc = m->eq_poly[r];
        float pos = QPOS[a1] - Q0[a1], vel = QVEL[eq_i];
        if (eq_j >= 0) {
          const int a2 = m->eq_qadr2[r];
          const float xx = QPOS[a2] - Q0[a2];
          pos -= pc[0] + xx * (pc[1] + xx * (pc[2] + xx * (pc[3] + xx * pc[4])));
          eq_c = pc[1] + xx * (2.0f * pc[2] + xx * (3.0f * pc[3] + xx * 4.0f * pc[4]));
          vel -= eq_c * QVEL[eq_j];
        } else {
// ... 2 lines not shown
        row_params(m->eq_imp[r], pos, m->eq_invweight[r], vel, eq_D, eq_aref);
      }
    }
  }
  float pj[EQP_ROWS], pjar_s[EQP_ROWS], pjar_w[EQP_ROWS];
  int np_rows = 0;
  float* EQW = L + S::O_EQP;
  if constexpr (S::EQ) {
    np_rows = m->eqp_nrow;
#pragma unroll
    for (int r = 0; r < EQP_ROWS; r++) { pj[r] = 0.0f; pjar_s[r] = 0.0f; pjar_w[r] = 0.0f; }
    if (np_rows > 0) {
      auto row_c = [&](int r) { return (m->neqp > 1 && r >= m->eqp_row0[1]) ? 1 : 0; };
      if (lane < np_rows) {
        const int c = row_c(lane), k = lane - m->eqp_row0[c], b1 = m->eqp_b1[c], b2 = m->eqp_b2[c];
        float q1[4], q2[4], p1[3], p2[3], t[3];
        for (int a = 0; a < 4; a++) { q1[a] = XQUAT[a * NB + b1]; q2[a] = XQUAT[a * NB + b2]; }
        qrot(t, q1, m->eqp_a1[c]); for (int a = 0; a < 3; a++) p1[a] = XPOS[a * NB + b1] + t[a];
        qrot(t, q2, m->eqp_a2[c]); for (int a = 0; a < 3; a++) p2[a] = XPOS[a * NB + b2] + t[a];
        float w1[6] = {0, 0, 0, 0, 0, 0}, w2[6] = {0, 0, 0, 0, 0, 0}, cpos;
        if (k < 3) {
          const float e[3] = {k == 0 ? 1.0f : 0.0f, k == 1 ? 1.0f : 0.0f, k == 2 ? 1.0f : 0.0f};
          const float r1[3] = {p1[0] - ref[0], p1[1] - ref[1], p1[2] - ref[2]}, r2[3] = {p2[0] - ref[0], p2[1] - ref[1], p2[2] - ref[2]};
          cross3(w1, r1, e); cross3(w2, r2, e);
          for (int a = 0; a < 3; a++) { w1[3 + a] = e[a]; w2[3 + a] = e[a]; }
          cpos = (k == 0 ? p1[0] - p2[0] : (k == 1 ? p1[1] - p2[1] : p1[2] - p2[2]));
        } else {
          const int kk = k - 3;
          const float ts = m->eqp_ts[c];
          float quat[4], q2c[4] = {q2[0], -q2[1], -q2[2], -q2[3]}, qe[4];
          qmul(quat, q1, m->eqp_relq[c]);
          qmul(qe, q2c, quat);
          cpos = (kk == 0 ? qe[1] : (kk == 1 ? qe[2] : qe[3])) * ts;
          for (int a = 0; a < 3; a++) {
            const float ax[4] = {0.0f, a == 0 ? 1.0f : 0.0f, a == 1 ? 1.0f : 0.0f, a == 2 ? 1.0f : 0.0f};
            float q3[4], q4[4];
            qmul(q3, q2c, ax); qmul(q4, q3, quat);
            const float v = 0.5f * ts * (kk == 0 ? q4[1] : (kk == 1 ? q4[2] : q4[3]));
            w1[a] = v; w2[a] = v;
          }
        }
        for (int a = 0; a < 6; a++) { EQW[S::EQP_W + 12 * lane + a] = w1[a]; EQW[S::EQP_W + 12 * lane + 6 + a] = w2[a]; }
        EQW[S::EQP_POS + lane] = cpos;
      }
      ODK_SYNC();
      float cdv[6];
#pragma unroll
      for (int k = 0; k < 6; k++) cdv[k] = st.d_on ? CDOF[k * NR + st.d_red] : 0.0f;
      const int pmask = st.d_on ? m->dof_eqp[lane] : 0;
      const float qv_l = st.d_on ? QVEL[lane] : 0.0f;
      float vr[EQP_ROWS];
#pragma unroll
      for (int r = 0; r < EQP_ROWS; r++) {
        float J = 0.0f;
        if (r < np_rows) {
          const int c = row_c(r);
          const float* w = EQW + S::EQP_W + 12 * r;
          float d1 = 0.0f, d2 = 0.0f;
#pragma unroll
          for (int k = 0; k < 6; k++) { d1 = fmaf(w[k], cdv[k], d1); d2 = fmaf(w[6 + k], cdv[k], d2); }
          J = (((pmask >> (2 * c)) & 1) ? d1 : 0.0f) - (((pmask >> (2 * c + 1)) & 1) ? d2 : 0.0f);
          if (st.d_on) EQW[S::EQP_J + r * NV + lane] = J;
        }
        pj[r] = J; vr[r] = J * qv_l;
      }
      gsum_n<G, EQP_ROWS>(vr);
      if (lane < np_rows) {
        const int c = row_c(lane), k = lane - m->eqp_row0[c];
        const int r0 = m->eqp_row0[c], r1 = (c + 1 < m->neqp) ? m->eqp_row0[c + 1] : np_rows;
        float nrm = 0.0f;
        for (int r = r0; r < r1; r++) { const float x = EQW[S::EQP_POS + r]; nrm = fmaf(x, x, nrm); }
        nrm = sqrtf(nrm);
        float vel = 0.0f;
#pragma unroll
        for (int r = 0; r < EQP_ROWS; r++) vel = r == lane ? vr[r] : vel;
        float D, aref;
        row_params_imp(m->eqp_imp[c], EQW[S::EQP_POS + lane], nrm, m->eqp_invw[c][k < 3 ? 0 : 1], vel, D, aref);
        EQW[S::EQP_D + lane] = D; EQW[S::EQP_AREF + lane] = aref;
      }
      ODK_SYNC();
    }
  }
  const bool ff_rows = __builtin_amdgcn_ballot_w64(fminf(fminf(CDIST[8], CDIST[9]), fminf(CDIST[10], CDIST[11])) < 0.0f) != 0;
  const bool prim_feet = !HF && m->foot_prim != 0;
  const bool ell = S::CONE || (S::ELL && m->cone != 0);
  for (int rc = lane; rc < S::NCROW; rc += G) {
    const int r = r0c + rc, c = rc >> 2, s = rc & 3, pair = c >> 2;
    if (rc >= 32 && !ff_rows) { ED[r] = 0.0f; AREF[r] = 0.0f; continue; }
    const float dist = CDIST[c];
    const float mu = CT[pair];
    const float fs = (s & 1) ? -mu : mu;
    const float* fr = (pair == 2 && dist < 0) ? SCR + S::S_VF : ((pair < 2 && (HF || prim_feet)) ? SCR + S::S_FR + 9 * c : CT + 33);
    const int td = 3 * (1 + (s >> 1));
    float dir[3] = {fr[0] + fs * fr[td], fr[1] + fs * fr[td + 1], fr[2] + fs * fr[td + 2]};
    if constexpr (S::ELL) {
      if (ell) {
        const float on3 = s < 3 ? 1.0f : 0.0f;
        const int ax = s < 3 ? 3 * s : 0;
        dir[0] = on3 * fr[ax]; dir[1] = on3 * fr[ax + 1]; dir[2] = on3 * fr[ax + 2];
      }
    }
    const float rr[3] = {CR[3 * c], CR[3 * c + 1], CR[3 * c + 2]};
    float ang[3];
    cross3(ang, rr, dir);
    float* wr = W + 6 * rc;
    wr[0] = ang[0]; wr[1] = ang[1]; wr[2] = ang[2]; wr[3] = dir[0]; wr[4] = dir[1]; wr[5] = dir[2];
    float D = 0, aref = 0;
    if (dist < 0) {
      float vel = 0;
      const int b2 = m->foot_body[pair == 0 ? 0 : 1];
#pragma unroll
      for (int k = 0; k < 6; k++) vel += wr[k] * CVEL[k * NB + b2];
      if (pair == 2) {
        const int b1 = m->foot_body[0];
#pragma unroll
        for (int k = 0; k < 6; k++) vel -= wr[k] * CVEL[k * NB + b1];
      }
      row_params(CT + 6 + 9 * pair, dist, CT[3 + pair], vel, D, aref);
      if constexpr (S::ELL) {
        if (ell) {
          if (s == 0) {  }
          else if (s < 3) { float Dn, an; row_params(CT + 6 + 9 * pair, dist, CT[3 + pair], 0.0f, Dn, an); D = Dn * m->impratio; aref = -CT[6 + 9 * pair + 1] * vel; }
          else { D = 0.0f; aref = 0.0f; }
        }
      }
    }
    ED[r] = D;
    AREF[r] = aref;
  }
  ODK_SYNC();
  ODK_PROF(9);

  gather_M();
  const float warm = st.d_on ? WARM[lane] : 0.0f;
  const float* VBQ = QAS; const float* VBW = WARM;
  if constexpr (S::PAIRED) {
    if (st.r_on) { X[lane] = pair_sum<S>(QAS, m, lane); MA[lane] = pair_sum<S>(WARM, m, lane); }
    ODK_SYNC();
    VBQ = X; VBW = MA;
  }
  auto foot_twist = [&](const float* V, int k, int f) -> float {
    float s = 0;
    if constexpr (S::CL > 0) {
      const int c0 = f ? m->foot_rchain_first[1] : m->foot_rchain_first[0], cl = f ? m->foot_rchain_len[1] : m->foot_rchain_len[0];
      const float* cd = CDOF + k * NR;
#pragma unroll
      for (int t = 0; t < 6; t++) s += cd[t] * V[t];
#pragma unroll
      for (int t = 0; t < S::CL; t++) { const float a = cd[c0 + t] * V[c0 + t]; s += t < cl ? a : 0.0f; }
    } else {
#pragma unroll
      for (int d = 0; d < NR; d++) {
        const int fm = ubcast(st.r_foot, d);
        const float vd = V[d];
        if ((fm >> f) & 1) s += CDOF[k * NR + d] * vd;
      }
    }
    return s;
  };
  {
    const int which = (lane / 12) & 1, f = (lane / 6) & 1, k = lane % 6;
    const float s = foot_twist(which ? VBW : VBQ, k, f);
    if (lane < 24) SCR[(which ? S::S_VF2 : S::S_VF) + 6 * f + k] = s;
  }
  const float ma_w = mul_M(VBW, MV, warm);
  const float gw = st.d_on ? (ma_w - qfs) * (warm - qas) : 0.0f;
  ODK_SYNC();
  auto contact_jx = [&](int rc, const float* VF) -> float {
    const int pair = rc >> 4;
    const float* wr = W + 6 * rc;
    const float* v2 = VF + (pair == 0 ? 0 : 6);
    float s = 0;
#pragma unroll
    for (int k = 0; k < 6; k++) s += wr[k] * v2[k];
    if (pair == 2) {
#pragma unroll
      for (int k = 0; k < 6; k++) s -= wr[k] * VF[k];
    }
    return s;
  };
  auto quad_cost = [](float D, float jar, float& force) -> float {
    if (D > 0 && jar < 0) { force = -D * jar; return 0.5f * D * jar * jar; }
    force = 0;
    return 0.0f;
  };
  auto fl_cost = [&](float jar, float& force) -> float {
    const float aj = fabsf(jar);
    const bool lin = aj >= fl_rf;
    force = lin ? (jar > 0 ? -fl_f : fl_f) : -fs.D * jar;
    return lin ? fl_f * (aj - 0.5f * fl_rf) : 0.5f * fs.D * jar * jar;
  };
  float cost_s = 0, cost_w = 0, jar_fl_s = 0, jar_fl_w = 0, jar_lim_s = 0, jar_lim_w = 0, fo;
  if (lane < nfl) {
    const float ar = AREF[lane];
    jar_fl_s = QAS[fs.dof] - ar; jar_fl_w = WARM[fs.dof] - ar;
    cost_s += fl_cost(jar_fl_s, fo); cost_w += fl_cost(jar_fl_w, fo);
  }
  float lim_D = 0.0f;
  if (st.d_lim_on) {
    const int r = nfl + st.d_limrow;
    lim_D = ED[r];
    const float ar = AREF[r];
    jar_lim_s = lim_sgn * qas - ar; jar_lim_w = lim_sgn * warm - ar;
    cost_s += quad_cost(lim_D, jar_lim_s, fo); cost_w += quad_cost(lim_D, jar_lim_w, fo);
  }
  float jar_eq_s = 0.0f, jar_eq_w = 0.0f;
  if constexpr (S::EQ) {
    if (eq_on) {
      jar_eq_s = QAS[eq_i] - eq_aref; jar_eq_w = WARM[eq_i] - eq_aref;
      if (eq_j >= 0) { jar_eq_s -= eq_c * QAS[eq_j]; jar_eq_w -= eq_c * WARM[eq_j]; }
      if (eq_first) { cost_s += 0.5f * eq_D * jar_eq_s * jar_eq_s; cost_w += 0.5f * eq_D * jar_eq_w * jar_eq_w; }
    }
  }
  if constexpr (S::EQ) {
    if (np_rows > 0) {
      float a9[EQP_ROWS], b9[EQP_ROWS];
#pragma unroll
      for (int r = 0; r < EQP_ROWS; r++) { a9[r] = pj[r] * qas; b9[r] = pj[r] * warm; }
      gsum_n<G, EQP_ROWS>(a9); gsum_n<G, EQP_ROWS>(b9);
#pragma unroll
      for (int r = 0; r < EQP_ROWS; r++) {
        if (r < np_rows) {
          const float ar = EQW[S::EQP_AREF + r], D = EQW[S::EQP_D + r];
          pjar_s[r] = a9[r] - ar; pjar_w[r] = b9[r] - ar;
          if (lane == r) { cost_s += 0.5f * D * pjar_s[r] * pjar_s[r]; cost_w += 0.5f * D * pjar_w[r] * pjar_w[r]; }
        }
      }
// ... 107 lines not shown
            if constexpr (S::ELL) v[q++] = ell ? w[a] * u[b2] : aw * w[b2];
            else v[q++] = aw * w[b2];
          }
        }
      }
#pragma unroll
      for (int q = 0; q < 27; q++) {
        float x = v[q];
        x += ODK_DPP(x, 0xB1, 0xF); x += ODK_DPP(x, 0x4E, 0xF); x += ODK_DPP(x, 0x141, 0xF); x += ODK_DPP(x, 0x140, 0xF);
        asm volatile("" : "+v"(x));
        v[q] = x;
      }
      if (on && (lane & 15) == 0) {
        const int blk = rc >> 4;
        float* FFb = SCR + (blk < 2 ? S::S_FF + 6 * blk : S::S_FFX);
        float* Kb = SCR + S::S_K + 36 * blk;
#pragma unroll
        for (int k = 0; k < 6; k++) FFb[k] = v[k];
        int q = 6;
#pragma unroll
        for (int a = 0; a < 6; a++)
#pragma unroll
          for (int b2 = a; b2 < 6; b2++) { Kb[6 * a + b2] = v[q]; Kb[6 * b2 + a] = v[q]; q++; }
      }
    }
    ODK_SYNC();
    if (!any_ff) {
      for (int t2 = lane; t2 < 36; t2 += G) SCR[S::S_K + 72 + t2] = 0.0f;
    } else {
      for (int t2 = lane; t2 < 36; t2 += G) { const float kx = SCR[S::S_K + 72 + t2]; SCR[S::S_K + t2] += kx; SCR[S::S_K + 36 + t2] += kx; }
      if (lane < 6) { const float fx = SCR[S::S_FFX + lane]; SCR[S::S_FF + lane] -= fx; SCR[S::S_FF + 6 + lane] += fx; }
    }
  }
  ODK_SYNC();
  const bool ff_active = c_act[2] && (SCR[S::S_K + 72 + 21] != 0.0f || SCR[S::S_K + 72 + 28] != 0.0f || SCR[S::S_K + 72 + 35] != 0.0f);
  float grad = 0.0f;
  if (st.d_on) {
    const int i = lane;
    float qc = 0, hdiag_extra = 0.0f;
    if (st.d_flrow >= 0) { qc += MV[i]; hdiag_extra += MA[i]; }
    if (st.d_lim_on) { qc += lim_sgn * f_lim; if (lim_D > 0 && jar_lim < 0) hdiag_extra += lim_D; }
    if constexpr (S::EQ) {
      if (eq_on) {
        const float je = eq_first ? 1.0f : -eq_c;
        qc += je * (-eq_D * jar_eq);
        hdiag_extra += eq_D * je * je;
        if (eq_first) SCR[S::S_EQ + eq_r] = -eq_D * eq_c;
      }
      if (np_rows > 0) {
#pragma unroll
        for (int r = 0; r < EQP_ROWS; r++) if (r < np_rows) qc += pj[r] * (-EQW[S::EQP_D + r] * pjar_s[r]);
      }
    }
    float cd[6];
#pragma unroll
    for (int k = 0; k < 6; k++) cd[k] = CDOF[k * NR + st.d_red];
#pragma unroll
    for (int f = 0; f < 2; f++)
      if ((st.d_foot >> f) & 1) {
#pragma unroll
        for (int k = 0; k < 6; k++) qc += cd[k] * SCR[S::S_FF + 6 * f + k];
      }
    grad = ma - qfs - qc;
    if (S::CL == 0 && st.d_tkind != 2) {
#pragma unroll
      for (int f = 0; f < 2; f++) {
        float* T = f ? BUF6B : BUF6;
        const bool on = ((st.d_foot >> f) & 1) && (c_act[f] || c_act[2]);
#pragma unroll
        for (int a = 0; a < 6; a++) {
          float s = 0;
          if (on) {
#pragma unroll
            for (int b2 = 0; b2 < 6; b2++) s += SCR[S::S_K + 36 * f + 6 * a + b2] * cd[b2];
          }
          T[a * NR + st.d_red] = s;
        }
      }
    }
    JV[i] = hdiag_extra;
  }
  if constexpr (S::CL > 0) {
    const int f = lane >= 6 + S::CL ? 1 : 0, idx = lane - (6 + S::CL) * f;
    const int c0 = f ? m->foot_rchain_first[1] : m->foot_rchain_first[0], cl = f ? m->foot_rchain_len[1] : m->foot_rchain_len[0];
    const bool lane_on = lane < 2 * (6 + S::CL) && idx - 6 < cl;
    const int col = lane_on ? (idx < 6 ? idx : c0 + idx - 6) : 0;
    const bool on = lane_on && ((f ? c_act[1] : c_act[0]) || c_act[2]);
    float cdc[6];
#pragma unroll
    for (int b2 = 0; b2 < 6; b2++) cdc[b2] = CDOF[b2 * NR + col];
    const float* Kf = SCR + S::S_K + 36 * f;
    float* T = f ? BUF6B : BUF6;
#pragma unroll
    for (int a = 0; a < 6; a++) {
      float s0 = 0.0f;
#pragma unroll
      for (int b2 = 0; b2 < 6; b2++) s0 = fmaf(Kf[6 * a + b2], cdc[b2], s0);
      if (lane_on) T[a * NR + col] = on ? s0 : 0.0f;
    }
  }
  ODK_SYNC();
  ODK_PROF(11);
  const bool any_ffa = __builtin_amdgcn_ballot_w64(ff_active) != 0 || (S::EQ && m->eqp_cross != 0);
  auto hess_entry = [&](int e, float v) -> float {
    const int i = e & 31, j = (e >> 5) & 31, fi = (e >> 10) & 3, fj = (e >> 12) & 3;
    if ((e >> 14) & 1) {
      const int u = (e >> 16) & 31;
      v += (S::PAIRED && ((e >> 15) & 1)) ? pair_einv(ARM, JV, u) : JV[u];
    }
    if constexpr (S::EQ) {
      for (int r = 0; r < m->neq; r++) v += (e & 0x3FF) == m->eq_key[r] ? SCR[S::S_EQ + r] : 0.0f;
      for (int r = 0; r < np_rows; r++) v = fmaf(EQW[S::EQP_D + r] * EQW[S::EQP_J + r * NV + i], EQW[S::EQP_J + r * NV + j], v);
    }
    const int both = fi & fj;
    if (both) {
      float cj[6];
#pragma unroll
      for (int k = 0; k < 6; k++) cj[k] = CDOF[k * NR + j];
      if (both & 1) {
#pragma unroll
        for (int k = 0; k < 6; k++) v += cj[k] * BUF6[k * NR + i];
      }
      if (both & 2) {
#pragma unroll
        for (int k = 0; k < 6; k++) v += cj[k] * BUF6B[k * NR + i];
      }
    }
    return v;
  };
  if (st.d_on) { if constexpr (DBG) MA[lane] = grad; GRAD[lane] = grad; }
  float rhs = grad;
  if constexpr (S::PAIRED) {
    ODK_SYNC();
    rhs = pair_rhs<S>(GRAD, ARM, JV, m, lane);
  }
  float search;
  if (!any_ffa) {
    {
      static_assert(G >= 21, "base x base entries must sit in the first pass");
      int ee[ST::NME]; float mm[ST::NME], hv[ST::NME];
#pragma unroll
      for (int t = 0; t < ST::NME; t++) { const int p = lane + t * G, pc = p < S::NMR ? p : 0; ee[t] = RT[pc]; mm[t] = M[pc]; }
#pragma unroll
      for (int t = 0; t < ST::NME; t++) {
        const int e = ee[t], i = e & 31, j = (e >> 5) & 31, both = (e >> 10) & (e >> 12) & 3, u = (e >> 16) & 31;
        float dterm = JV[u];
        if constexpr (S::PAIRED) { const float pe = pair_einv(ARM, JV, u); dterm = ((e >> 15) & 1) ? pe : dterm; }
        float cj[6];
#pragma unroll
        for (int k = 0; k < 6; k++) cj[k] = CDOF[k * NR + j];
        const float* T1 = (both & 1) ? BUF6 : BUF6B;
        float s1 = 0.0f;
#pragma unroll
        for (int k = 0; k < 6; k++) s1 = fmaf(cj[k], T1[k * NR + i], s1);
        float v = mm[t] + (((e >> 14) & 1) ? dterm : 0.0f) + (both ? s1 : 0.0f);
        if constexpr (S::EQ) {
          for (int r = 0; r < m->neq; r++) v += (e & 0x3FF) == m->eq_key[r] ? SCR[S::S_EQ + r] : 0.0f;
          for (int r = 0; r < np_rows; r++) v = fmaf(EQW[S::EQP_D + r] * EQW[S::EQP_J + r * NV + i], EQW[S::EQP_J + r * NV + j], v);
        }
        if (t == 0) {
          float s2 = 0.0f;
#pragma unroll
          for (int k = 0; k < 6; k++) s2 = fmaf(cj[k], BUF6B[k * NR + i], s2);
          v += both == 3 ? s2 : 0.0f;
        }
        hv[t] = v;
      }
// ... 37 lines not shown
          const float wgt = (float)(((fi >> 1) & 1) && (fj & 1)) + (float)((fi & 1) && ((fj >> 1) & 1));
          if (wgt != 0.0f) {
            float sx = 0;
            for (int a2 = 0; a2 < 6; a2++)
              for (int b2 = 0; b2 < 6; b2++) sx += CDOF[a2 * NR + i] * SCR[S::S_K + 72 + 6 * a2 + b2] * CDOF[b2 * NR + j];
            v -= wgt * sx;
          }
        }
        HL[lane + t * G] = v;
      }
    }
    ODK_SYNC();
    ODK_PROF(12);
    factor_rows<G, S::DVR, NR>(HL, lane, st.r_on, v_depth, v_Madr, v_descmask, v_depth, v_Madr);
    ODK_PROF(13);
    const float z = solve_rows<G, NR>(HL, rhs, lane, st.r_on, v_depth, v_Madr, v_ancmask, v_descmask, v_depth, v_Madr);
    if constexpr (S::PAIRED) {
      if (st.r_on) MV[lane] = z;
      ODK_SYNC();
      search = -pair_expand<S, G>(MV, GRAD, grad, ARM, JV, st, lane);
    } else {
      search = -z;
    }
    ODK_PROF(14);
  }

  ODK_SYNC();
  if (st.d_on) GRAD[lane] = search;
  ODK_SYNC();
  const float* VBS = GRAD;
  if constexpr (S::PAIRED) {
    if (st.r_on) X[lane] = pair_sum<S>(GRAD, m, lane);
    ODK_SYNC();
    VBS = X;
  }
  const float mv = mul_M(VBS, MV, search);
  float sn = st.d_on ? search * search : 0.0f, qg1 = st.d_on ? search * (ma - qfs) : 0.0f, qg2 = st.d_on ? 0.5f * search * mv : 0.0f;
  { float r3[3] = {sn, qg1, qg2}; gsum_n<G, 3>(r3); sn = r3[0]; qg1 = r3[1]; qg2 = r3[2]; }
  ODK_SYNC();
  {
    const float s = foot_twist(VBS, lane % 6, (lane / 6) & 1);
    if (lane < 12) SCR[S::S_VF + lane] = s;
  }
  ODK_SYNC();
  float jv_fl = 0, jv_lim = 0;
  if (lane < nfl) jv_fl = GRAD[fs.dof];
  if (st.d_lim_on) jv_lim = lim_sgn * search;
  float jv_eq = 0.0f, eq_Dw = 0.0f;
  float pr_D = 0.0f, pr_jar = 0.0f, pr_jv = 0.0f;
  if constexpr (S::EQ) {
    if (eq_on && eq_first) { jv_eq = GRAD[eq_i] - (eq_j >= 0 ? eq_c * GRAD[eq_j] : 0.0f); eq_Dw = eq_D; }
    if (np_rows > 0) {
      float s9[EQP_ROWS];
#pragma unroll
      for (int r = 0; r < EQP_ROWS; r++) s9[r] = st.d_on ? pj[r] * search : 0.0f;
      gsum_n<G, EQP_ROWS>(s9);
#pragma unroll
      for (int r = 0; r < EQP_ROWS; r++) if (r == lane && r < np_rows) { pr_D = EQW[S::EQP_D + r]; pr_jar = pjar_s[r]; pr_jv = s9[r]; }
    }
  }
#pragma unroll
  for (int t = 0; t < NCL; t++) {
    const int rc = lane + t * G;
    const bool on = rc < S::NCROW;
    cjv[t] = 0.0f;
    if (!(t * G >= 32 && !any_ff)) cjv[t] = (on && cD[t] > 0) ? contact_jx(rc, SCR + S::S_VF) : 0.0f;
    if constexpr (DBG) { if (on) JV[r0c + rc] = cjv[t]; }
  }
  ODK_PROF(15);
  float ls_x[NCL][3], ls_v[NCL][3], ls_Dn[NCL], ls_Dt[NCL], ls_Dm[NCL], ls_mu[NCL], ls_mur[NCL], ls_on[NCL];
  if constexpr (S::ELL) {
    if (ell) {
#pragma unroll
      for (int t = 0; t < NCL; t++) {
        const int rc = lane + t * G;
        quad3(cjar[t], ls_x[t]); quad3(cjv[t], ls_v[t]);
        ls_Dn[t] = ODK_DPP(cD[t], 0x00, 0xF);
        ls_mu[t] = CT[(rc < S::NCROW ? rc : 0) >> 4];
        ls_mur[t] = ls_mu[t] * ell_mur; ls_Dt[t] = ls_Dn[t] * m->impratio; ls_Dm[t] = cone_dm(ls_Dn[t], ls_mur[t]);
        ls_on[t] = ((rc & 3) < 3 && rc < S::NCROW) ? 1.0f : 0.0f;
      }
    }
  }
  const float gtol = m->tolerance * m->ls_tolerance * sqrtf(sn) * m->meaninertia * (float)(NV > 1 ? NV : 1);
  auto ls_eval = [&](auto cost_tag, const float* al, float* cost, float* d0, float* d1) {
    constexpr bool COST = decltype(cost_tag)::value;
    float acc[9] = {0, 0, 0, 0, 0, 0, 0, 0, 0};
    {
      const float D = fs.D, jar = jar_fl, jv = jv_fl;
      const float q0 = 0.5f * D * jar * jar, q1 = D * jv * jar, q2 = 0.5f * D * jv * jv;
      const float lo0 = fl_f * (-0.5f * fl_rf - jar), lo1 = -fl_f * jv, hi0 = fl_f * (-0.5f * fl_rf + jar), hi1 = fl_f * jv;
#pragma unroll
      for (int a = 0; a < 3; a++) {
        const float xx = jar + al[a] * jv;
        const bool lo = xx <= -fl_rf, hi = xx >= fl_rf;
        if constexpr (COST) acc[3 * a] = lo ? lo0 : (hi ? hi0 : q0);
        acc[3 * a + 1] = lo ? lo1 : (hi ? hi1 : q1); acc[3 * a + 2] = (lo || hi) ? 0.0f : q2;
      }
    }
    {
      const float D = lim_D, jar = jar_lim, jv = jv_lim;
      const float q0 = 0.5f * D * jar * jar, q1 = D * jv * jar, q2 = 0.5f * D * jv * jv;
#pragma unroll
      for (int a = 0; a < 3; a++) {
        const float w = jar + al[a] * jv < 0 ? 1.0f : 0.0f;
        if constexpr (COST) acc[3 * a] = fmaf(w, q0, acc[3 * a]);
        acc[3 * a + 1] = fmaf(w, q1, acc[3 * a + 1]); acc[3 * a + 2] = fmaf(w, q2, acc[3 * a + 2]);
      }
    }
    if constexpr (S::EQ) {
      const float D = eq_Dw, jar = jar_eq, jv = jv_eq;
      const float q0 = 0.5f * D * jar * jar + 0.5f * pr_D * pr_jar * pr_jar, q1 = D * jv * jar + pr_D * pr_jv * pr_jar, q2 = 0.5f * D * jv * jv + 0.5f * pr_D * pr_jv * pr_jv;
#pragma unroll
      for (int a = 0; a < 3; a++) {
        if constexpr (COST) acc[3 * a] += q0;
        acc[3 * a + 1] += q1; acc[3 * a + 2] += q2;
      }
    }
#pragma unroll
    for (int t = 0; t < NCL; t++) {
      if (t * G >= 32 && !any_ff) continue;
      if constexpr (S::ELL) {
        if (ell) {
          const int sa = lane & 3;
          const float als = sa == 0 ? al[0] : (sa == 1 ? al[1] : al[2]);
          const float xx[3] = {ls_x[t][0] + als * ls_v[t][0], ls_x[t][1] + als * ls_v[t][1], ls_x[t][2] + als * ls_v[t][2]};
          float cc, d0c, d1c;
          cone_line(ls_Dn[t], ls_Dt[t], ls_Dm[t], ls_mu[t], ls_mur[t], xx, ls_v[t], cc, d0c, d1c);
          const float t1c = d0c - als * d1c, t2c = 0.5f * d1c;
#pragma unroll
          for (int a = 0; a < 3; a++) {
            const float w = sa == a ? ls_on[t] : 0.0f;
            if constexpr (COST) acc[3 * a] = fmaf(w, cc, acc[3 * a]);
            else { acc[3 * a + 1] = fmaf(w, t1c, acc[3 * a + 1]); acc[3 * a + 2] = fmaf(w, t2c, acc[3 * a + 2]); }
          }
          continue;
        }
      }
      const float D = cD[t], jar = cjar[t], jv = cjv[t];
      const float q0 = 0.5f * D * jar * jar, q1 = D * jv * jar, q2 = 0.5f * D * jv * jv;
#pragma unroll
      for (int a = 0; a < 3; a++) {
        const float w = jar + al[a] * jv < 0 ? 1.0f : 0.0f;
        if constexpr (COST) acc[3 * a] = fmaf(w, q0, acc[3 * a]);
        acc[3 * a + 1] = fmaf(w, q1, acc[3 * a + 1]); acc[3 * a + 2] = fmaf(w, q2, acc[3 * a + 2]);
      }
    }
    if constexpr (COST) {
      float c[3];
#pragma unroll
      for (int a = 0; a < 3; a++) c[a] = fmaf(al[a], fmaf(al[a], acc[3 * a + 2], acc[3 * a + 1]), acc[3 * a]);
      gsum_n<G, 3>(c);
#pragma unroll
      for (int a = 0; a < 3; a++) cost[a] = c[a] + fmaf(al[a], fmaf(al[a], qg2, qg1), gauss);
    } else {
      float r[6] = {acc[1], acc[2], acc[4], acc[5], acc[7], acc[8]};
      gsum_n<G, 6>(r);
#pragma unroll
      for (int a = 0; a < 3; a++) {
        const float t1 = r[2 * a] + qg1, t2 = r[2 * a + 1] + qg2;
        d0[a] = 2.0f * al[a] * t2 + t1;
        d1[a] = 2.0f * t2 + (t2 == 0.0f ? MINVAL_F : 0.0f);
      }
    }
  };
  using Deriv = std::integral_constant<bool, false>; using Cost = std::integral_constant<bool, true>;
  auto sdiv = [](float a, float b) { return b == 0.0f ? 0.0f : a * __builtin_amdgcn_rcpf(b); };
  float al[3] = {0, 0, 0}, cs[3], e0[3], e1[3];
  ls_eval(Deriv(), al, cs, e0, e1);
  const float p0_d0 = e0[0], p0_d1 = e1[0];
  al[0] = -sdiv(p0_d0, p0_d1); al[1] = al[0]; al[2] = al[0];
  ls_eval(Deriv(), al, cs, e0, e1);
  float lo_a, lo_d0, lo_d1, hi_a, hi_d0, hi_d1;
  if (e0[0] < p0_d0) { lo_a = al[0]; lo_d0 = e0[0]; lo_d1 = e1[0]; hi_a = 0; hi_d0 = p0_d0; hi_d1 = p0_d1; }
  else { hi_a = al[0]; hi_d0 = e0[0]; hi_d1 = e1[0]; lo_a = 0; lo_d0 = p0_d0; lo_d1 = p0_d1; }
  bool swap = true;
  for (int it = 0; it < m->ls_iterations; it++) {
    bool done = !swap || (lo_d0 < 0 && lo_d0 > -gtol) || (hi_d0 > 0 && hi_d0 < gtol);
    if (done) break;
    al[0] = lo_a - sdiv(lo_d0, lo_d1); al[1] = hi_a - sdiv(hi_d0, hi_d1); al[2] = 0.5f * (lo_a + hi_a);
    ls_eval(Deriv(), al, cs, e0, e1);
    const bool s1 = (lo_d0 > 0) || (lo_d0 < e0[0]);
    if (s1) { lo_a = al[0]; lo_d0 = e0[0]; lo_d1 = e1[0]; }
    const bool s2 = (e0[2] < 0) && (lo_d0 < e0[2]);
    if (s2) { lo_a = al[2]; lo_d0 = e0[2]; lo_d1 = e1[2]; }
    const bool s3 = (e0[1] < 0) && (lo_d0 < e0[1]);
    if (s3) { lo_a = al[1]; lo_d0 = e0[1]; lo_d1 = e1[1]; }
    const bool s4 = (hi_d0 < 0) || (hi_d0 > e0[1]);
    if (s4) { hi_a = al[1]; hi_d0 = e0[1]; hi_d1 = e1[1]; }
    const bool s5 = (e0[2] > 0) && (hi_d0 > e0[2]);
    if (s5) { hi_a = al[2]; hi_d0 = e0[2]; hi_d1 = e1[2]; }
    const bool s6 = (e0[0] > 0) && (hi_d0 > e0[0]);
    if (s6) { hi_a = al[0]; hi_d0 = e0[0]; hi_d1 = e1[0]; }
    swap = s1 || s2 || s3 || s4 || s5 || s6;
  }
  al[0] = lo_a; al[1] = hi_a; al[2] = 0.0f;
  ls_eval(Cost(), al, cs, e0, e1);
  const float lo_c = cs[0], hi_c = cs[1], p0_cost = cs[2];
  const bool improved = (lo_c < p0_cost) || (hi_c < p0_cost);
  const float alpha = improved ? (lo_c < hi_c ? lo_a : hi_a) : 0.0f;
  if (st.d_on) {
    const float xa = x + alpha * search;
    X[lane] = xa;
    WARM[lane] = xa;
  }
  if constexpr (DBG) {
    if (lane == 0) { SCR[S::S_MISC + 13] = qg1; SCR[S::S_MISC + 14] = qg2; SCR[S::S_MISC + 15] = gauss; }
    if (lane == 0) { SCR[S::S_MISC + 4] = p0_d0; SCR[S::S_MISC + 5] = p0_d1; SCR[S::S_MISC + 6] = p0_cost; SCR[S::S_MISC + 7] = gtol; }
    if (lane == 0) { SCR[S::S_MISC + 1] = alpha; SCR[S::S_MISC + 2] = use_warm ? 1.0f : 0.0f; SCR[S::S_MISC + 3] = use_warm ? cost_w : cost_s; }
  }
  ODK_SYNC();
  ODK_PROF(16);

  if (flags & 1) {
    if (lane < m->nsensor) {
      const int s = lane, site = m->sensor_site[s], b = m->site_body[site], type = m->sensor_type[s];
      float R[9], Rs[9], sp[3], dif[3], qb[4];
      for (int k = 0; k < 4; k++) qb[k] = XQUAT[k * NB + b];
      q2mat(R, qb);
      for (int i = 0; i < 3; i++)
        for (int j = 0; j < 3; j++) Rs[3 * i + j] = R[3 * i] * m->site_mat[site][j] + R[3 * i + 1] * m->site_mat[site][3 + j] + R[3 * i + 2] * m->site_mat[site][6 + j];
      for (int k = 0; k < 3; k++) {
        sp[k] = XPOS[k * NB + b] + R[3 * k] * m->site_pos[site][0] + R[3 * k + 1] * m->site_pos[site][1] + R[3 * k + 2] * m->site_pos[site][2];
        dif[k] = sp[k] - ref[k];
      }
      float cv[6];
      for (int k = 0; k < 6; k++) cv[k] = CVEL[k * NB + b];
      float vang[3] = {cv[0], cv[1], cv[2]}, t[3], vlin[3];
      cross3(t, dif, vang);
      vlin[0] = cv[3] - t[0]; vlin[1] = cv[4] - t[1]; vlin[2] = cv[5] - t[2];
      float* out = SENS + m->sensor_adr[s];
      auto tmul = [&](float* o, const float* v) {
        o[0] = Rs[0] * v[0] + Rs[3] * v[1] + Rs[6] * v[2];
        o[1] = Rs[1] * v[0] + Rs[4] * v[1] + Rs[7] * v[2];
        o[2] = Rs[2] * v[0] + Rs[5] * v[1] + Rs[8] * v[2];
      };
      if (type == 0) tmul(out, vang);
      else if (type == 1) tmul(out, vlin);
      else if (type == 2) {
        float ca[6];
        for (int k = 0; k < 6; k++) ca[k] = CACC[k * NB + b];
        for (int d = 0; d < 6; d++) {
          const float qa = X[d];
          for (int k = 0; k < 6; k++) ca[k] += CDOF[k * NR + d] * qa;
        }
        float al3[3], wl[3], vl[3], corr[3], acc[3];
        cross3(t, dif, ca);
        al3[0] = ca[3] - t[0]; al3[1] = ca[4] - t[1]; al3[2] = ca[5] - t[2];
        tmul(acc, al3); tmul(wl, vang); tmul(vl, vlin);
        cross3(corr, wl, vl);
        out[0] = acc[0] + corr[0]; out[1] = acc[1] + corr[1]; out[2] = acc[2] + corr[2];
      } else if (type == 3) { out[0] = Rs[2]; out[1] = Rs[5]; out[2] = Rs[8]; }
      else if (type == 4) { out[0] = Rs[0]; out[1] = Rs[3]; out[2] = Rs[6]; }
      else if (type == 5) { out[0] = vlin[0]; out[1] = vlin[1]; out[2] = vlin[2]; }
      else if (type == 6) { out[0] = vang[0]; out[1] = vang[1]; out[2] = vang[2]; }
      else if (type == 7) { out[0] = sp[0]; out[1] = sp[1]; out[2] = sp[2]; }
      else if (type == 8) {
        float qs[4];
        qmul(qs, qb, m->site_quat[site]);
        qnormalize(qs);
// ... 49 lines not shown
```

open_duck_playground_amd/csrc/odk_model.h:

```cpp
#pragma once
#include <stdint.h>

namespace odk {

constexpr int EQ_MAX = 2;
constexpr int EQP_MAX = 2, EQP_ROWS = 9;
constexpr int MAXV = 32;
constexpr int MAXQ = 32;
constexpr int MAXB = 20;
constexpr int MAXJ = 26;
constexpr int MAXU = 16;
constexpr int MAXNZ = 512;
constexpr int MAXHV = 20;
constexpr int MAXHF = 40;
constexpr int MAXHE = 64;
constexpr int HULL_MAXV = 17;
constexpr int HULL_MAXF = 30;
constexpr int HULL_MAXE = 48;
static_assert(HULL_MAXV <= MAXHV && HULL_MAXF <= MAXHF && HULL_MAXE <= MAXHE && HULL_MAXF <= 32 && HULL_MAXE <= 48 && HULL_MAXV <= 17, "kernel hull regions");
constexpr int MAXCHAIN = 8;
constexpr int MAXSITE = 8;
constexpr int MAXSENS = 16;
constexpr int NCON = 12;
constexpr int NSENSD = 46;

struct BodySt {
  int level, parent, child[4], njnt, jd[2], jj[2], jr[2], pathmask, is_path, upmask, path_head;
  float pos[3], quat[4], ipos[3], inertia[6], ax[2][3];
  int body;
};

struct LaneSt {
  int j_qadr, j_dadr;
  int cs_pk;
  int ch_first, ch_len;
  int r_on, r_depth, r_Madr, r_ancmask, r_descmask, r_foot;
  int m_adr[16];
  int d_on, d_body;
  int d_act, d_flrow, d_limrow, d_foot;
  int d_qadr, d_lim_on;
  int d_tkind, d_red;
  float d_damping, d_lo, d_hi;
};

struct ObsEnt { int a, b; float kc; int fl; };
constexpr int OBS_FL_VEL = 1 << 13, OBS_FL_PLUS0 = 1 << 14;
constexpr int OBS_MAX = 232;
constexpr int OBS_PARK_CON = 1, OBS_PARK_IMI = 3, OBS_PARK_PHASE = 4;

struct DevModel {
  BodySt body_st[2][64];
  LaneSt lane_st[64];
  int nq, nv, nu, nb, nj, nM, nH, nfl, nlim, nrow, nsite, nsensor;
  float dt, gravity[3], tolerance, ls_tolerance, impratio, meaninertia;
  int ls_iterations, iterations;
  int base_body, body_in_tree[MAXB], body_parent[MAXB], body_jntadr[MAXB], body_jntnum[MAXB];
  int max_level, body_level[MAXB], body_children[MAXB][4];
  int max_nonpath_level, body_pathmask[MAXB], body_is_path[MAXB], body_upmask[MAXB], body_path_head[MAXB];
  int np_count, np_body[4], np_nsrc[4], np_src[4][MAXB];
  int body_chain[MAXB][MAXCHAIN], body_chain_len[MAXB];
  int body_ancdof[MAXB][MAXV], body_nancdof[MAXB];
  int body_sub[MAXB][MAXB], body_nsub[MAXB];
  float body_pos[MAXB][3], body_quat[MAXB][4], body_ipos[MAXB][3], body_mass[MAXB], body_inertia[MAXB][6];
  int jnt_qposadr[MAXJ], jnt_dofadr[MAXJ], jnt_bodyid[MAXJ];
  float jnt_axis[MAXJ][3], jnt_pos[MAXJ][3], jnt_range[MAXJ][2], qpos0[MAXQ];
  int dof_body[MAXV], dof_depth[MAXV], dof_anc[MAXV][MAXV], dof_Madr[MAXV], dof_anc_adr[MAXV][MAXV];
  int dof_ndesc[MAXV], dof_desc[MAXV][MAXV], dof_desc_adr[MAXV][MAXV];
  int dof_nprefix[MAXV], dof_prefix[MAXV][MAXV];
  int dof_nsym[MAXV], dof_sym_dof[MAXV][MAXV], dof_sym_adr[MAXV][MAXV];
  int dof_act[MAXV], dof_flrow[MAXV], dof_limrow[MAXV];
  int dof_ancmask[MAXV], dof_descmask[MAXV], vdof_ancmask[MAXV], vdof_descmask[MAXV];
  int dof_qadr[MAXV], dof_jnt[MAXV];
  float dof_range[MAXV][2];
  float dof_armature[MAXV], dof_damping[MAXV], dof_frictionloss[MAXV], dof_invweight0[MAXV];
  int M_i[MAXNZ], M_j[MAXNZ];
  int M_ent[MAXNZ];
  int pad_chains[7];
  int paired, nvr, nMr, nHr;
  int dof_tkind[MAXV];
  int dof_red[MAXV];
  int red_main[MAXV], red_twin[MAXV];
  int red_depth[MAXV], red_Madr[MAXV], red_ancmask[MAXV], red_descmask[MAXV], red_foot[MAXV];
  int rv_depth[MAXV], rv_Madr[MAXV], rv_ancmask[MAXV], rv_descmask[MAXV];
  int nrchain; short rchain_first[4], rchain_len[4]; int pad_rchain[2];
  int foot_rchain_first[2], foot_rchain_len[2];
  int R_ent[MAXNZ], RH_ent[MAXNZ];
  int vdof_depth[MAXV], vdof_anc[MAXV][MAXV], vdof_Madr[MAXV], vdof_anc_adr[MAXV][MAXV];
  int vdof_ndesc[MAXV], vdof_desc[MAXV][MAXV], vdof_desc_adr[MAXV][MAXV];
  int H_i[MAXNZ], H_j[MAXNZ], H_src[MAXNZ];
  int tri_m[MAXNZ], tri_q[MAXNZ];
  int act_qposadr[MAXU], act_dofadr[MAXU], act_backlash_qposadr[MAXU];
  float act_kp[MAXU], act_bias1[MAXU], act_bias2[MAXU], act_ctrlrange[MAXU][2], act_forcerange[MAXU][2];
  int act_ctrllimited[MAXU], act_forcelimited[MAXU];
  float key_qpos[MAXQ], key_ctrl[MAXU];
  int fl_dof[MAXV], lim_jnt[MAXJ];
  float fl_D[MAXV], fl_R[MAXV], fl_b[MAXV];
  float lim_solref[MAXJ][2], lim_solimp[MAXJ][5], lim_invweight[MAXJ];
  float pair_solref[3][2], pair_solimp[3][5], pair_mu[3], pair_invweight[3];
  float lim_imp[MAXJ][9], pair_imp[3][9];
  int foot_body[2], foot_nvert[2], foot_nface[2], foot_dofmask[2][MAXV];
  float foot_vert[2][MAXHV][3];
  int foot_face[2][MAXHF][3];
  float foot_obb_center[2][3], foot_obb_half[2][3], foot_obb_axes[2][9];
  float foot_sphere_r[2];
  int foot_npoly[2], foot_nedge[2];
  int foot_poly[2][MAXHF][5];
  float foot_fnorm[2][MAXHF][3];
  float foot_foff[2][MAXHF];
  int foot_edge[2][MAXHE][4];
  int foot_lane_rec[2][16][8];
  float foot_centroid[2][3];
  int foot_prim, foot_gtype[2];
  float foot_gpos[2][3], foot_gaxis[2][3], foot_gsize[2][3];
  float plane_pos[3], plane_n[3], plane_frame[9];
  int floor_is_plane;
  int hfield_nrow, hfield_ncol;
  float hfield_size[4], floor_mat[9];
  int hfield_filter;
  int site_body[MAXSITE], site_imu, site_feet[2];
  float site_pos[MAXSITE][3], site_mat[MAXSITE][9], site_quat[MAXSITE][4];
  int sensor_type[MAXSENS], sensor_site[MAXSENS], sensor_adr[MAXSENS];
  int adr_gyro, adr_local_linvel, adr_accelerometer, adr_upvector, adr_global_angvel, adr_foot_linvel[2];
  int eqp_cross;
  int neqp, eqp_nrow, eqp_type[EQP_MAX], eqp_b1[EQP_MAX], eqp_b2[EQP_MAX], eqp_row0[EQP_MAX], dof_eqp[MAXV];
  float eqp_a1[EQP_MAX][3], eqp_a2[EQP_MAX][3], eqp_relq[EQP_MAX][4], eqp_ts[EQP_MAX], eqp_imp[EQP_MAX][9], eqp_invw[EQP_MAX][2];
  int cone;
  int neq, eq_dof1[EQ_MAX], eq_dof2[EQ_MAX], eq_qadr1[EQ_MAX], eq_qadr2[EQ_MAX], eq_key[EQ_MAX], dof_eqrow[MAXV];
  float eq_poly[EQ_MAX][5], eq_imp[EQ_MAX][9], eq_invweight[EQ_MAX];
  alignas(16) ObsEnt obs_tab[2][OBS_MAX];
};

constexpr int PRISM_EDGE[9][4] = {{0, 1, 0, 2}, {1, 2, 0, 3}, {3, 5, 1, 4}, {0, 3, 2, 4}, {3, 4, 2, 1}, {1, 4, 3, 2}, {4, 5, 3, 1}, {2, 5, 4, 3}, {0, 2, 4, 0}};
constexpr int PRISM_POLY[5][5] = {{3, 0, 1, 2, 0}, {3, 3, 5, 4, 3}, {4, 0, 3, 4, 1}, {4, 1, 4, 5, 2}, {4, 2, 5, 3, 0}};

struct HfAssign { int v[625]; };
constexpr HfAssign make_hf_assign() {
  HfAssign T{};
  for (int idx = 0; idx < 625; idx++) {
    const int c[4] = {idx % 5, (idx / 5) % 5, (idx / 25) % 5, idx / 125};
    int asg[4] = {0, 0, 0, 0}, tgt[4] = {0, 1, 2, 3}, rnk[4] = {0, 0, 0, 0}, on[4] = {0, 0, 0, 0};
    for (int r = 0; r < 4; r++) if (c[r] > 0) { asg[r] = 1; on[r] = 1; }
    for (int r = 0; r < 4; r++) {
      if (on[r]) continue;
      int bt = -1, bl = 0;
      for (int t = 0; t < 4; t++) if (c[t] - asg[t] > bl) { bl = c[t] - asg[t]; bt = t; }
      if (bt >= 0) { tgt[r] = bt; rnk[r] = asg[bt]; asg[bt]++; on[r] = 1; }
    }
    int mq = 1;
    for (int t = 0; t < 4; t++) mq = asg[t] > mq ? asg[t] : mq;
    unsigned w = 0;
    for (int r = 0; r < 4; r++) w |= (unsigned)tgt[r] << (2 * r) | (unsigned)rnk[r] << (8 + 2 * r) | (unsigned)on[r] << (16 + r);
    T.v[idx] = (int)(w | (unsigned)(mq - 1) << 20);
  }
  return T;
}

struct DevPRM {
  int nx, ny, nth, nsteps;
  float dxs[16], dys[16], dths[16], ranges[6];
};

}
```

open_duck_playground_amd/csrc/odk_model_load.hip:

```cpp
#include <stddef.h>
#include <stdint.h>

#include <cmath>
#include <cstdarg>
#include <cstdio>
#include <cstdlib>
#include <cstring>
#include <array>
#include <memory>
#include <string>
#include <vector>

#define ODK_HOST_ONLY
#include "odk_host.h"
#include "odk_obs_layout.h"
#include "odk_shapes.h"

using namespace odk;

static thread_local std::string g_err;
int odk::fail(int code, const char* fmt, ...) {
  char buf[512];
  va_list ap;
  va_start(ap, fmt);
// ... 800 lines not shown
}

int load_equalities(Load& c) {
  DevModel& m = c.m;
  const bool shape_ok = c.shape_eq && !m.paired;
  m.neq = 0;
  for (int d = 0; d < MAXV; d++) m.dof_eqrow[d] = -1;
  m.neqp = 0; m.eqp_nrow = 0; m.eqp_cross = 0;
  for (int d = 0; d < MAXV; d++) m.dof_eqp[d] = 0;
  for (int pass = 0; pass < 2; pass++)
    for (int k = 0; k < c.eq_n; k++) {
      if (!c.eq_active[k] || c.eq_type[k] != pass) continue;
      const char* kind = pass == 0 ? "connect" : "weld";
      const int nrow = pass == 0 ? 3 : 6;
      if (!shape_ok || m.neqp == EQP_MAX || m.eqp_nrow + nrow > EQP_ROWS)
        return fail(ODK_ERR_UNSUPPORTED, "<equality><%s> (constraint %d) is active: %s", kind, k,
                    shape_ok ? "the kernels hold at most two connect / weld constraints with nine rows in total" : NO_EQ_ROWS);
      const int q = m.neqp, b1 = c.eq_o1[k], b2 = c.eq_o2[k] < 0 ? 0 : c.eq_o2[k];
      if (b1 < 1 || b1 >= m.nb || b2 >= m.nb) return fail(ODK_ERR_UNSUPPORTED, "<equality><%s> (constraint %d): bad body ids", kind, k);
      unsigned above[2] = {0u, 0u};
      for (int s2 = 0; s2 < 2; s2++)
        for (int b = s2 ? b2 : b1; b > 0; b = m.body_parent[b])
          for (int d = 0; d < m.nv; d++) if (m.dof_body[d] == b) above[s2] |= 1u << d;
      if ((above[0] & above[1]) != above[0] && (above[0] & above[1]) != above[1]) {
        unsigned legs = 0x3Fu;
        for (int f = 0; f < 2; f++) for (int t = 0; t < m.foot_rchain_len[f]; t++) legs |= 1u << (m.foot_rchain_first[f] + t);
        if (((above[0] | above[1]) & ~legs) != 0u || m.paired)
          return fail(ODK_ERR_UNSUPPORTED, "<equality><%s> (constraint %d): the two bodies must lie on one root-to-leaf path of the tree (or body2 be the world), or on the two foot chains: another loop has no entries in the Hessian's layouts", kind, k);
        m.eqp_cross = 1;
      }
      for (int d = 0; d < m.nv; d++) m.dof_eqp[d] |= (((above[0] >> d) & 1) << (2 * q)) | (((above[1] >> d) & 1) << (2 * q + 1));
      const double* da = c.eq_data + 11 * k;
      for (int a = 0; a < 3; a++) { m.eqp_a1[q][a] = (float)(pass == 0 ? da[a] : da[3 + a]); m.eqp_a2[q][a] = (float)(pass == 0 ? da[3 + a] : da[a]); }
      for (int a = 0; a < 4; a++) m.eqp_relq[q][a] = pass == 0 ? (a == 0 ? 1.0f : 0.0f) : (float)da[6 + a];
      m.eqp_ts[q] = pass == 0 ? 0.0f : (float)da[10];
      eq_pack_imp(c, k, m.eqp_imp[q]);
      m.eqp_invw[q][0] = (float)(c.biw[2 * b1] + c.biw[2 * b2]); m.eqp_invw[q][1] = (float)(c.biw[2 * b1 + 1] + c.biw[2 * b2 + 1]);
      m.eqp_type[q] = pass; m.eqp_b1[q] = b1; m.eqp_b2[q] = b2; m.eqp_row0[q] = m.eqp_nrow;
      m.eqp_nrow += nrow; m.neqp++;
    }
  for (int k = 0; k < c.eq_n; k++) {
    if (!c.eq_active[k] || c.eq_type[k] != 2) continue;
    if (!shape_ok || m.neq == EQ_MAX)
      return fail(ODK_ERR_UNSUPPORTED, "<equality><joint> (constraint %d) is active: %s", k, shape_ok ? "the kernels hold at most two equality rows" : NO_EQ_ROWS);
    const int r = m.neq, j1 = c.eq_o1[k], j2 = c.eq_o2[k];
    if (j1 < 1 || j1 >= m.nj || j2 >= m.nj || j2 == 0 || j2 == j1) return fail(ODK_ERR_UNSUPPORTED, "<equality><joint> (constraint %d): hinge joints expected", k);
    const int d1 = m.jnt_dofadr[j1], d2 = j2 > 0 ? m.jnt_dofadr[j2] : -1;
    if (m.dof_eqrow[d1] >= 0 || (d2 >= 0 && m.dof_eqrow[d2] >= 0)) return fail(ODK_ERR_UNSUPPORTED, "<equality><joint> (constraint %d): a joint takes part in at most one equality row", k);
    m.eq_dof1[r] = d1; m.eq_dof2[r] = d2; m.eq_qadr1[r] = m.jnt_qposadr[j1]; m.eq_qadr2[r] = j2 > 0 ? m.jnt_qposadr[j2] : 0;
    m.eq_key[r] = -1;
    if (d2 >= 0) {
      for (int p = 0; p < m.nMr; p++) {
        const int e = m.R_ent[p], i = e & 31, j = (e >> 5) & 31;
        if ((i == d1 && j == d2) || (i == d2 && j == d1)) m.eq_key[r] = e & 0x3FF;
      }
      if (m.eq_key[r] < 0) return fail(ODK_ERR_UNSUPPORTED, "<equality><joint> (constraint %d): the two joints must lie on one serial chain (the coupling's Hessian term needs an entry of the tree layout)", k);
    }
    for (int a = 0; a < 5; a++) m.eq_poly[r][a] = (float)c.eq_data[11 * k + a];
    eq_pack_imp(c, k, m.eq_imp[r]);
    m.eq_invweight[r] = (float)(c.dof_iw[d1] + (d2 >= 0 ? c.dof_iw[d2] : 0.0));
    m.dof_eqrow[d1] = r; if (d2 >= 0) m.dof_eqrow[d2] = r;
    m.neq++;
  }
  return 0;
}

int build_statics(Load& c) {
  DevModel& m = c.m;
  const int shape = c.mo.shape;
  if (shape == 1 && !(m.paired && m.nvr == ShapeB::NVR && m.nMr == ShapeB::NMR && m.nHr == ShapeB::NHR))
    return fail(ODK_ERR_UNSUPPORTED, "the 30-dof kernels expect backlash twins (same body, anchor and axis as their joint) over the 20-dof tree");
  if (shape != 1 && m.paired) return fail(ODK_ERR_UNSUPPORTED, "twin dofs in a model of the 20-dof shape");
  for (int lane = 0; lane < 64; lane++) {
    memset(&m.lane_st[lane], 0, sizeof(LaneSt));
#define X(i, S) if (shape == i) compute_statics<S>(m.lane_st[lane], &m, lane);
    ODK_SHAPES(X)
#undef X
  }
#define X(i, S) if (shape == i) build_obs_table<S>(m);
  ODK_SHAPES(X)
#undef X
  return 0;
}
}

extern "C" int odk_model_load(const void* blob, uint64_t len, odk_model** out) {
  if (!blob || !out || len < 16 || memcmp(blob, "ODKM", 4) != 0) return fail(ODK_ERR_INVALID, "odk_model_load: not an ODKM blob");
  Blob B;
  if (const char* bad = B.open((const unsigned char*)blob, len)) return fail(ODK_ERR_INVALID, "odk_model_load: record %d: %s", (int)B.recs.size(), bad);
  auto mo = std::make_unique<odk_model>();
  memset(&mo->h, 0, sizeof(mo->h));
  Load c{B, *mo, mo->h};
  int (*const stages[])(Load&) = {load_options, collect_equalities, load_tree,        load_actuators, load_rows,       load_feet,
                                  load_floor,   load_sensors,       build_fold_lists, select_shape,   load_equalities, build_statics};
  for (auto stage : stages)
    if (const int err = stage(c)) return err;
  *out = mo.release();
  return ODK_OK;
}
extern "C" void odk_model_free(odk_model* m) { delete m; }
extern "C" int odk_model_dims(const odk_model* m, int* nq, int* nv, int* nu, int* nbody) {
  if (!m) return fail(ODK_ERR_INVALID, "null model");
  if (nq) *nq = m->h.nq; if (nv) *nv = m->h.nv; if (nu) *nu = m->h.nu; if (nbody) *nbody = m->h.nb;
  return ODK_OK;
}
extern "C" int odk_model_obs_sizes(const odk_model* m, int env_kind, int* nobs, int* npriv) {
  if (!m) return fail(ODK_ERR_INVALID, "null model");
  obs_sizes_nu(m->h.nu, env_kind, nobs, npriv);
  return ODK_OK;
}
extern "C" int odk_model_reduced(const odk_model* m, int* paired, int* nvr, int* nMr, int* nHr, int* red_main, int* red_twin) {
  if (!m) return fail(ODK_ERR_INVALID, "null model");
  if (paired) *paired = m->h.paired; if (nvr) *nvr = m->h.nvr; if (nMr) *nMr = m->h.nMr; if (nHr) *nHr = m->h.nHr;
  for (int r = 0; r < m->h.nvr; r++) { if (red_main) red_main[r] = m->h.red_main[r]; if (red_twin) red_twin[r] = m->h.red_twin[r]; }
  return ODK_OK;
}
extern "C" int odk_model_body_lanes(const odk_model* m, int lanes_per_env, int* out, int n) {
  if (!m || !out || (lanes_per_env != 32 && lanes_per_env != 64)) return fail(ODK_ERR_INVALID, "odk_model_body_lanes: bad arguments");
  for (int l = 0; l < n && l < lanes_per_env; l++) out[l] = m->h.body_st[lanes_per_env == 64][l].body;
  return ODK_OK;
}
extern "C" int odk_model_env_lds_floats(const odk_model* m) {
  if (!m) return -1;
#define X(i, S) if (m->shape == i) return EnvL<S>::TOTAL;
  ODK_SHAPES(X)
#undef X
  return -1;
}
```

open_duck_playground_amd/engine.py:

```python
from __future__ import annotations

import ctypes as C
import os
import subprocess
from typing import Dict, List, Optional

import numpy as np

from .model import Model, asset_path

_CSRC = os.path.join(os.path.dirname(os.path.abspath(__file__)), "csrc")
LIB_PATH = os.environ.get("ODK_LIB", os.path.join(_CSRC, "libodk.so"))

NOBS, NPRIV, NMETRIC, NU = 101, 212, 8, 14
ADAM_ACC_FLOATS = 2 + 1024
METRIC_NAMES = ("reward/tracking_lin_vel", "reward/tracking_ang_vel", "cost/torques", "cost/action_rate", "cost/stand_still",
                "reward/alive", "reward/imitation", "swing_peak")

XTERM_NAMES = ("lin_vel_z", "ang_vel_xy", "orientation", "base_height", "energy", "joint_pos_limits", "termination", "pose", "feet_slip",
               "feet_clearance", "feet_height", "feet_air_time")
NXTERM = len(XTERM_NAMES)

PARAM_BODY_MASS, PARAM_BODY_IPOS_TORSO, PARAM_DOF_FRICTIONLOSS, PARAM_DOF_ARMATURE, PARAM_QPOS0, PARAM_KP = range(6)

# ... 290 lines not shown
    _check_placement(name, acc, torch.float32, device)


def _check_report(batch, name: str, acc, ncol: int, track_acc) -> None:
    check_accumulator(f"{name}: acc", acc, batch.nenv, ncol, batch.device)
    check_accumulator(f"{name}: track_acc", track_acc, batch.nenv, TRACK_NACC, batch.device)


def _report_ptrs(batch, track_acc):
    return tuple(C.c_void_p(t.data_ptr()) for t in (batch.priv, batch.done, batch.truncation, track_acc))


def _check_torque_limit(batch, name: str, t):
    if t is None:
        return None
    if not hasattr(t, "dim") or t.dim() != 1:
        raise OdkError(f"{name}: torque_limit: expected a 1-D torch tensor or None, got {type(t).__name__}")
    check_accumulator(f"{name}: torque_limit", t.unsqueeze(0), 1, batch.model.nu, batch.device)
    return C.c_void_p(t.data_ptr())


def check_schedule(name: str, sched, sched_of_env, nenv: int, device: int):
    import torch
    if not torch.is_tensor(sched):
        raise OdkError(f"{name}: sched: expected a torch tensor, got {type(sched).__name__}")
    if sched.dim() != 3 or int(sched.shape[0]) < 1 or not 1 <= int(sched.shape[1]) <= SCHED_MAX_SEGMENTS or int(sched.shape[2]) != SCHED_SEG_FLOATS:
        raise OdkError(f"{name}: sched: shape must be (nsched >= 1, 1 .. {SCHED_MAX_SEGMENTS}, {SCHED_SEG_FLOATS}), got {tuple(sched.shape)}")
    _check_placement(f"{name}: sched", sched, torch.float32, device)
    if not torch.is_tensor(sched_of_env):
        raise OdkError(f"{name}: sched_of_env: expected a torch tensor, got {type(sched_of_env).__name__}")
    if tuple(sched_of_env.shape) != (int(nenv),):
        raise OdkError(f"{name}: sched_of_env: shape must be ({nenv},), got {tuple(sched_of_env.shape)}")
    _check_placement(f"{name}: sched_of_env", sched_of_env, torch.int32, device)
    return int(sched.shape[0]), int(sched.shape[1])


def _chk(rc: int):
    if rc != 0:
        raise OdkError(f"odk error {rc}: {load_library().odk_last_error().decode()}")


def default_config(standing: bool = False) -> EnvConfig:
    cfg = EnvConfig()
    L = load_library()
    (L.odk_default_config_standing if standing else L.odk_default_config)(C.byref(cfg))
    return cfg


def obs_sizes(env_kind: int):
    a, b = C.c_int(0), C.c_int(0)
    load_library().odk_obs_sizes(int(env_kind), C.byref(a), C.byref(b))
    return a.value, b.value


def model_obs_sizes(model: Model, env_kind: int = 0):
    L = load_library()
    blob = model.blob()
    h = C.c_void_p()
    _chk(L.odk_model_load(blob, len(blob), C.byref(h)))
    try:
        a, b = C.c_int(0), C.c_int(0)
        _chk(L.odk_model_obs_sizes(h, int(env_kind), C.byref(a), C.byref(b)))
        return a.value, b.value
    finally:
        L.odk_model_free(h)


def model_reduction(model: Model) -> Dict:
    L = load_library()
    blob = model.blob()
    h = C.c_void_p()
    _chk(L.odk_model_load(blob, len(blob), C.byref(h)))
    try:
        ints = [C.c_int(0) for _ in range(4)]
        main, twin = (C.c_int * 32)(), (C.c_int * 32)()
        _chk(L.odk_model_reduced(h, *[C.byref(i) for i in ints], main, twin))
        nvr = ints[1].value
        return dict(paired=ints[0].value, nvr=nvr, nMr=ints[2].value, nHr=ints[3].value, main=list(main)[:nvr], twin=list(twin)[:nvr],
                    env_lds_floats=L.odk_model_env_lds_floats(h))
    finally:
        L.odk_model_free(h)


def model_body_lanes(model: Model, lanes_per_env: int) -> List[int]:
    L = load_library()
    blob = model.blob()
    h = C.c_void_p()
    _chk(L.odk_model_load(blob, len(blob), C.byref(h)))
    try:
        out = (C.c_int * lanes_per_env)()
        _chk(L.odk_model_body_lanes(h, int(lanes_per_env), out, lanes_per_env))
        return list(out)
    finally:
        L.odk_model_free(h)


def load_prm() -> Dict[str, np.ndarray]:
    z = np.load(asset_path("prm_table.npz"))
    return {k: z[k] for k in z.files}


def _fp(a: np.ndarray):
    return a.ctypes.data_as(C.POINTER(C.c_float))


def _dp(a: np.ndarray):
    return a.ctypes.data_as(C.POINTER(C.c_double))


def _stream(t):
    import torch
    return C.c_void_p(torch.cuda.current_stream(t.device).cuda_stream)


def _ptr(t):
    return C.c_void_p(t.data_ptr()) if t is not None else None


def _f32c(*ts):
    for t in ts:
        if t is not None and not (t.is_cuda and t.is_contiguous() and t.dtype.is_floating_point and t.element_size() == 4):
            raise OdkError("learner kernels take contiguous float32 CUDA tensors")


def gae(truncation, termination, rewards, values, bootstrap, lambda_: float, discount: float, vs=None, adv=None, stats=None):
    import torch
    B, T = rewards.shape
    vs = torch.empty_like(rewards) if vs is None else vs
    adv = torch.empty_like(rewards) if adv is None else adv
    _f32c(truncation, termination, rewards, values, bootstrap, vs, adv, stats)
    _chk(load_library().odk_gae(_ptr(truncation), _ptr(termination), _ptr(rewards), _ptr(values), _ptr(bootstrap), _ptr(vs), _ptr(adv),
                                _ptr(stats), B, T, lambda_, discount, _stream(rewards)))
    return vs, adv


def ppo_head(logits, raw_action, old_log_prob, adv, stats, vs, baseline, noise, dlogits, dbaseline, losses, clipping_epsilon: float,
             entropy_cost: float, grad_scale: float = 1.0):
    n, a2 = logits.shape
    _f32c(logits, raw_action, old_log_prob, adv, stats, vs, baseline, noise, dlogits, dbaseline, losses)
    _chk(load_library().odk_ppo_head(_ptr(logits), _ptr(raw_action), _ptr(old_log_prob), _ptr(adv), _ptr(stats), _ptr(vs), _ptr(baseline),
                                     _ptr(noise), _ptr(dlogits), _ptr(dbaseline), _ptr(losses), n, a2 // 2, clipping_epsilon, entropy_cost,
                                     grad_scale, _stream(logits)))


def adam_clip(params, grads, m, v, acc, lr: float, max_grad_norm: float = 0.0, b1: float = 0.9, b2: float = 0.999, eps: float = 1e-8):
    _f32c(params, grads, m, v, acc)
    if acc.numel() < ADAM_ACC_FLOATS:
        raise OdkError("adam_clip: acc needs ADAM_ACC_FLOATS floats")
    _chk(load_library().odk_adam_clip(_ptr(params), _ptr(grads), _ptr(m), _ptr(v), _ptr(acc), params.numel(), lr, b1, b2, eps,
                                      max_grad_norm or 0.0, _stream(params)))


def policy_sample(logits, noise, out=None):
    import torch
    n, A = noise.shape
    _f32c(logits, noise)
    if out is not None:
        raw, act, logp = out
        _f32c(raw, act, logp)
        if raw.numel() != n * A or act.numel() != n * A or logp.numel() != n:
            raise OdkError("policy_sample: out tensors of the wrong size")
    else:
        raw, act, logp = torch.empty_like(noise), torch.empty_like(noise), torch.empty(n, device=noise.device)
    _chk(load_library().odk_policy_sample(_ptr(logits), _ptr(noise), _ptr(raw), _ptr(act), _ptr(logp), n, A, _stream(noise)))
    return raw, act, logp

# ... 653 lines not shown
```

Baseline: 20.61 million.

## Pack hot model scalars into SGPR words and LDS to cut global loads

```diff
diff --git a/include/odk.h b/include/odk.h
--- a/include/odk.h
+++ b/include/odk.h
@@ -76,6 +76,7 @@
 int odk_model_reduced(const odk_model* m, int* paired, int* nvr, int* nMr, int* nHr, int* red_main, int* red_twin);
 int odk_model_body_lanes(const odk_model* m, int lanes_per_env, int* out, int n);
 int odk_model_env_lds_floats(const odk_model* m);
+int odk_model_hot_words(const odk_model* m, int* packed, int* fields);
 
 int odk_batch_create(const odk_model* m, const odk_env_config* cfg, int nenv, int device, const float* prm_table,
                      const double* dxs, int nx, const double* dys, int ny, const double* dths, int nth, const double* ranges6,
diff --git a/open_duck_playground_amd/csrc/odk_env_kernels.h b/open_duck_playground_amd/csrc/odk_env_kernels.h
--- a/open_duck_playground_amd/csrc/odk_env_kernels.h
+++ b/open_duck_playground_amd/csrc/odk_env_kernels.h
@@ -6,7 +6,7 @@
 
 
 
-template <class S> __device__ __forceinline__ const int* load_shared(float* lds, int envs, const DevModel* m) {
+template <class S, bool HOT = false> __device__ __forceinline__ const int* load_shared(float* lds, int envs, const DevModel* m) {
   int* RT = reinterpret_cast<int*>(lds + envs * EnvL<S>::TOTAL);
   {
     constexpr int T = (S::NMR + 63) / 64;
@@ -22,6 +22,9 @@
   if (k < 3) { CT[k] = m->pair_mu[k]; CT[3 + k] = m->pair_invweight[k]; }
   if (k < 27) CT[6 + k] = m->pair_imp[k / 9][k % 9];
   if (k < 9) CT[33 + k] = m->plane_frame[k];
+  if constexpr (HOT && S::HOT_LDS) {
+    if (k < HOT_NF) SH[S::SH_HOT + k] = m->hot_f[k];
+  }
   return RT;
 }
 
@@ -388,7 +391,7 @@
   odk_poison_fill(lds, E::wg_floats(64 / G));
   ODK_SYNC();
 #endif
-  const int* RT = load_shared<S>(lds, 64 / G, a.m);
+  const int* RT = load_shared<S, HF == 0>(lds, 64 / G, a.m);
   const DevModel* m = a.m;
   const EnvCfg& c = a.cfg;
   float* INFO = L + E::O_INFO; float* ACT = L + E::O_ACT; float* CTRL = L + S::O_CTRL;
diff --git a/open_duck_playground_amd/csrc/odk_kernels.h b/open_duck_playground_amd/csrc/odk_kernels.h
--- a/open_duck_playground_amd/csrc/odk_kernels.h
+++ b/open_duck_playground_amd/csrc/odk_kernels.h
@@ -38,7 +38,7 @@
   static constexpr int NMR = PAIRED ? 145 : NM_;
   static constexpr int NHR = PAIRED ? 170 : NH_;
   static constexpr int DVR = PAIRED ? 15 : DV_;
-  static constexpr int SH_CT = NMR, SHARED = SH_CT + 42;
+  static constexpr int SH_CT = NMR, SH_HOT = SH_CT + 42;
   static constexpr int CL = CL_ >= 0 ? CL_ : ((NV_ == 20 || NV_ == 21 || PAIRED) ? 5 : 0);
   static constexpr int NCH = NCH_;
   static_assert(NCH >= 1 && NCH <= 4, "chain_solve: one 8-lane group per chain, 32 lanes");
@@ -107,6 +107,9 @@
   static constexpr int TOTAL = O_WX + (W_FITS ? 0 : 6 * NCROW);
   static constexpr int N_INFO = ((43 + 7 * NU + 3) / 4) * 4, N_ACT = ((NU + 2 + 3) / 4) * 4;
   static constexpr int ENV_STRIDE = TOTAL + N_INFO + N_ACT;
+  static constexpr int wgs_per_cu(int floats) { return 163840 / (4 * floats) > 8 ? 8 : 163840 / (4 * floats); }
+  static constexpr bool HOT_LDS = wgs_per_cu(2 * ENV_STRIDE + SH_HOT + HOT_NF) == wgs_per_cu(2 * ENV_STRIDE + SH_HOT);
+  static constexpr int SHARED = SH_HOT + (HOT_LDS ? HOT_NF : 0);
 };
 
 #ifdef ODK_PROFILE
@@ -273,7 +276,7 @@
 struct ActSt { float bias2, clo, chi, flo, fhi; int climited, flimited; };
 struct FlSt { float D, R, b; int dof; };
 
-struct HotSt { ActSt as; FlSt fs; float vb[3]; };
+struct HotSt { ActSt as; FlSt fs; float vb[3], ve[3]; int pk[HOT_NPK], np[2]; };
 
 template <class S, int G>
 __device__ __forceinline__ void load_statics(Statics<S, G>& st, const DevModel* __restrict__ m, int lane) {
@@ -353,8 +356,12 @@
   load_fl(h.fs, m, lane);
   const int f = (lane >> 4) & 1, j = lane & 15;
   const int jv = (lane < 32 && j < m->foot_nvert[f]) ? j : 0;
-  for (int k = 0; k < 3; k++) h.vb[k] = m->foot_vert[f][jv][k];
-}
+  for (int k = 0; k < 3; k++) { h.vb[k] = m->foot_vert[f][jv][k]; h.ve[k] = m->foot_vert[f][16][k]; }
+  for (int k = 0; k < HOT_NPK; k++) h.pk[k] = m->hot_pk[k];
+  h.np[0] = m->np_rec[lane][0]; h.np[1] = m->np_rec[lane][1];
+}
+__device__ __forceinline__ float& lds_at(float* base, int byte_off) { return *reinterpret_cast<float*>(reinterpret_cast<char*>(base) + byte_off); }
+__device__ __forceinline__ const float& lds_at(const float* base, int byte_off) { return *reinterpret_cast<const float*>(reinterpret_cast<const char*>(base) + byte_off); }
 __device__ __forceinline__ int load_rent(const DevModel* __restrict__ m, int p, int n) { const int e = m->R_ent[p < n ? p : 0]; return p < n ? e : -1; }
 __device__ __forceinline__ int load_rhent(const DevModel* __restrict__ m, int p, int n) { const int e = m->RH_ent[p < n ? p : 0]; return p < n ? e : -1; }
 
@@ -1629,6 +1636,16 @@
 __device__ __forceinline__ void forward_env(float* L, const int* RT, const DevModel* __restrict__ m, const float* __restrict__ hfield, const Statics<S, G>& st, int lane, int flags, const HotSt& hot = HotSt()) {
   const float* SH = reinterpret_cast<const float*>(RT);
   const float* CT = SH + S::SH_CT;
+  int hpk[HOT_NPK] = {0, 0, 0};
+  if constexpr (PRE) {
+#pragma unroll
+    for (int k = 0; k < HOT_NPK; k++) { int w = hot.pk[k]; asm volatile("" : "+v"(w)); hpk[k] = __builtin_amdgcn_readfirstlane(w); }
+  }
+  constexpr bool HOTF = PRE && S::HOT_LDS;
+  const float* HOTV = SH + S::SH_HOT;
+#define ODK_HOTI(F, expr) (PRE ? hot_value(hpk, F) : (expr))
+#define ODK_HOTF(i, expr) (HOTF ? HOTV[i] : (expr))
+#define ODK_OBBC(f, k) ODK_HOTF(HOT_F_OBBC + 3 * (f) + (k), m->foot_obb_center[f][k])
   constexpr int NV = S::NV, NB = S::NB, NR = S::NVR;
   using ST = Statics<S, G>;
   float* QPOS = L + S::O_QPOS; float* QVEL = L + S::O_QVEL; float* WARM = L + S::O_WARM; float* CTRL = L + S::O_CTRL;
@@ -1675,7 +1692,7 @@
       for (int k = 0; k < 3; k++) p[k] = stat ? bs.pos[k] : 0.0f;
       for (int k = 0; k < 4; k++) q[k] = stat ? bs.quat[k] : (k == 0 ? 1.0f : 0.0f);
     }
-    const int max_np = m->max_nonpath_level;
+    const int max_np = ODK_HOTI(HOT_NP_LEVELS, m->max_nonpath_level + 1) - 1;
     for (int lvl = 0; lvl <= max_np; lvl++) {
       if (bs.level == lvl && !bs.is_path) {
         if (lvl == 0) {
@@ -1928,13 +1945,23 @@
   {
     float* ACC = CFRC;
     static_assert(S::O_CRB == S::O_CFRC + 6 * NB, "cfrc | crb must be contiguous");
-    const int nnp = m->np_count;
+    const int nnp = ODK_HOTI(HOT_NP_COUNT, m->np_count);
     const int slot = lane >> 4, q = lane & 15;
     float t[2] = {0.0f, 0.0f};
+    int np0 = 0, np1 = 0;
+    if constexpr (PRE) { np0 = hot.np[0]; np1 = hot.np[1]; asm volatile("" : "+v"(np0), "+v"(np1)); }
 #pragma unroll
     for (int pass = 0; pass < 2; pass++) {
       const int i = pass * (G / 16) + slot;
       if (i < nnp) {
+        if (PRE && pass == 0) {
+          const int ns = (int)((unsigned)np1 >> 24);
+          float x = 0.0f;
+#pragma unroll
+          for (int c = 0; c < 6; c++) { const float y = lds_at(ACC + q * NB, (int)(((unsigned)(c < 4 ? np0 : np1) >> (8 * (c & 3))) & 0xFFu)); x += c < ns ? y : 0.0f; }
+          t[pass] = x;
+          continue;
+        }
         const int ns = m->np_nsrc[i];
         int src[6];
 #pragma unroll
@@ -1949,7 +1976,10 @@
 #pragma unroll
     for (int pass = 0; pass < 2; pass++) {
       const int i = pass * (G / 16) + slot;
-      if (i < nnp) ACC[q * NB + m->np_body[i]] = t[pass];
+      if (i < nnp) {
+        if (PRE && pass == 0) lds_at(ACC + q * NB, (int)(((unsigned)np1 >> 16) & 0xFFu)) = t[pass];
+        else ACC[q * NB + m->np_body[i]] = t[pass];
+      }
     }
     ODK_SYNC();
   }
@@ -2072,7 +2102,7 @@
   float fR[2][9], fP[2][3];
 #pragma unroll
   for (int f = 0; f < 2; f++) {
-    const int fb = m->foot_body[f];
+    const int fb = PRE ? (f ? hot_value(hpk, HOT_FOOT_BODY1) : hot_value(hpk, HOT_FOOT_BODY0)) : m->foot_body[f];
     float q[4];
     for (int k = 0; k < 4; k++) q[k] = XQUAT[k * NB + fb];
     for (int k = 0; k < 3; k++) fP[f][k] = XPOS[k * NB + fb];
@@ -2081,16 +2111,16 @@
   if constexpr (HF) {
     if constexpr (HF == 2) { hfield_prim_floor<S, G>(L, m, hfield, lane); ODK_SYNC(); prim_contacts<S, G>(L, m, lane, false); }
     else hfield_contacts<S, G>(L, m, hfield, lane);
-  } else if (m->foot_prim) {
+  } else if (ODK_HOTI(HOT_FOOT_PRIM, m->foot_prim)) {
     prim_contacts<S, G>(L, m, lane, true);
   } else {
-  const float pn0[3] = {m->plane_n[0], m->plane_n[1], m->plane_n[2]};
+  const float pn0[3] = {ODK_HOTF(HOT_F_PLN, m->plane_n[0]), ODK_HOTF(HOT_F_PLN + 1, m->plane_n[1]), ODK_HOTF(HOT_F_PLN + 2, m->plane_n[2])};
   {
     const int f = (lane >> 4) & 1, j = lane & 15;
-    const int nvt = m->foot_nvert[f];
+    const int nvt = PRE ? (f ? hot_value(hpk, HOT_FOOT_NVERT1) : hot_value(hpk, HOT_FOOT_NVERT0)) : m->foot_nvert[f];
     const bool inrow = lane < 32;
     const bool has = inrow && j < nvt, has_e = inrow && nvt > 16;
-    float pn[3] = {pn0[0], pn0[1], pn0[2]}, pp[3] = {m->plane_pos[0], m->plane_pos[1], m->plane_pos[2]};
+    float pn[3] = {pn0[0], pn0[1], pn0[2]}, pp[3] = {ODK_HOTF(HOT_F_PLP, m->plane_pos[0]), ODK_HOTF(HOT_F_PLP + 1, m->plane_pos[1]), ODK_HOTF(HOT_F_PLP + 2, m->plane_pos[2])};
     float Rf[9], Pf[3];
 #pragma unroll
     for (int k = 0; k < 9; k++) Rf[k] = f ? fR[1][k] : fR[0][k];
@@ -2101,7 +2131,8 @@
       const int jv = has ? j : 0;
       float vb[3];
       if constexpr (PRE) { vb[0] = hot.vb[0]; vb[1] = hot.vb[1]; vb[2] = hot.vb[2]; } else { vb[0] = m->foot_vert[f][jv][0]; vb[1] = m->foot_vert[f][jv][1]; vb[2] = m->foot_vert[f][jv][2]; }
-      const float ve[3] = {m->foot_vert[f][16][0], m->foot_vert[f][16][1], m->foot_vert[f][16][2]};
+      float ve[3];
+      if constexpr (PRE) { ve[0] = hot.ve[0]; ve[1] = hot.ve[1]; ve[2] = hot.ve[2]; } else { ve[0] = m->foot_vert[f][16][0]; ve[1] = m->foot_vert[f][16][1]; ve[2] = m->foot_vert[f][16][2]; }
 #pragma unroll
       for (int k = 0; k < 3; k++) {
         w[k] = Pf[k] + Rf[3 * k] * vb[0] + Rf[3 * k + 1] * vb[1] + Rf[3 * k + 2] * vb[2];
@@ -2129,17 +2160,17 @@
   }
   }
   ODK_PROF(7);
-  if (!m->foot_prim) {
+  if (!ODK_HOTI(HOT_FOOT_PRIM, m->foot_prim)) {
     float sep = -3.0e38f;
     float sph;
     {
       float dc[3];
       for (int k = 0; k < 3; k++) {
-        const float a1 = fP[0][k] + fR[0][3 * k] * m->foot_obb_center[0][0] + fR[0][3 * k + 1] * m->foot_obb_center[0][1] + fR[0][3 * k + 2] * m->foot_obb_center[0][2];
-        const float a2 = fP[1][k] + fR[1][3 * k] * m->foot_obb_center[1][0] + fR[1][3 * k + 1] * m->foot_obb_center[1][1] + fR[1][3 * k + 2] * m->foot_obb_center[1][2];
+        const float a1 = fP[0][k] + fR[0][3 * k] * ODK_OBBC(0, 0) + fR[0][3 * k + 1] * ODK_OBBC(0, 1) + fR[0][3 * k + 2] * ODK_OBBC(0, 2);
+        const float a2 = fP[1][k] + fR[1][3 * k] * ODK_OBBC(1, 0) + fR[1][3 * k + 1] * ODK_OBBC(1, 1) + fR[1][3 * k + 2] * ODK_OBBC(1, 2);
         dc[k] = a2 - a1;
       }
-      sph = sqrtf(dot3(dc, dc)) - m->foot_sphere_r[0] - m->foot_sphere_r[1];
+      sph = sqrtf(dot3(dc, dc)) - ODK_HOTF(HOT_F_SPHR, m->foot_sphere_r[0]) - ODK_HOTF(HOT_F_SPHR + 1, m->foot_sphere_r[1]);
     }
     float boxsep = -3.0e38f;
     if (__builtin_amdgcn_ballot_w64(!(sph > 0.0f)) != 0) {
@@ -2148,7 +2179,7 @@
   #pragma unroll
         for (int f = 0; f < 2; f++) {
           float* cc = f ? c2 : c1; float* AA = f ? A2 : A1;
-          for (int k = 0; k < 3; k++) cc[k] = fP[f][k] + fR[f][3 * k] * m->foot_obb_center[f][0] + fR[f][3 * k + 1] * m->foot_obb_center[f][1] + fR[f][3 * k + 2] * m->foot_obb_center[f][2];
+          for (int k = 0; k < 3; k++) cc[k] = fP[f][k] + fR[f][3 * k] * ODK_OBBC(f, 0) + fR[f][3 * k + 1] * ODK_OBBC(f, 1) + fR[f][3 * k + 2] * ODK_OBBC(f, 2);
           for (int i = 0; i < 3; i++)
             for (int j = 0; j < 3; j++) AA[3 * i + j] = fR[f][3 * i] * m->foot_obb_axes[f][j] + fR[f][3 * i + 1] * m->foot_obb_axes[f][3 + j] + fR[f][3 * i + 2] * m->foot_obb_axes[f][6 + j];
         }
@@ -2317,7 +2348,7 @@
     }
   }
   const bool ff_rows = __builtin_amdgcn_ballot_w64(fminf(fminf(CDIST[8], CDIST[9]), fminf(CDIST[10], CDIST[11])) < 0.0f) != 0;
-  const bool prim_feet = !HF && m->foot_prim != 0;
+  const bool prim_feet = !HF && ODK_HOTI(HOT_FOOT_PRIM, m->foot_prim) != 0;
   const bool ell = S::CONE || (S::ELL && m->cone != 0);
   for (int rc = lane; rc < S::NCROW; rc += G) {
     const int r = r0c + rc, c = rc >> 2, s = rc & 3, pair = c >> 2;
@@ -2343,11 +2374,11 @@
     float D = 0, aref = 0;
     if (dist < 0) {
       float vel = 0;
-      const int b2 = m->foot_body[pair == 0 ? 0 : 1];
+      const int b2 = PRE ? (pair == 0 ? hot_value(hpk, HOT_FOOT_BODY0) : hot_value(hpk, HOT_FOOT_BODY1)) : m->foot_body[pair == 0 ? 0 : 1];
 #pragma unroll
       for (int k = 0; k < 6; k++) vel += wr[k] * CVEL[k * NB + b2];
       if (pair == 2) {
-        const int b1 = m->foot_body[0];
+        const int b1 = ODK_HOTI(HOT_FOOT_BODY0, m->foot_body[0]);
 #pragma unroll
         for (int k = 0; k < 6; k++) vel -= wr[k] * CVEL[k * NB + b1];
       }
@@ -2377,7 +2408,7 @@
   auto foot_twist = [&](const float* V, int k, int f) -> float {
     float s = 0;
     if constexpr (S::CL > 0) {
-      const int c0 = f ? m->foot_rchain_first[1] : m->foot_rchain_first[0], cl = f ? m->foot_rchain_len[1] : m->foot_rchain_len[0];
+      const int c0 = f ? ODK_HOTI(HOT_RCHAIN_FIRST1, m->foot_rchain_first[1]) : ODK_HOTI(HOT_RCHAIN_FIRST0, m->foot_rchain_first[0]), cl = f ? ODK_HOTI(HOT_RCHAIN_LEN1, m->foot_rchain_len[1]) : ODK_HOTI(HOT_RCHAIN_LEN0, m->foot_rchain_len[0]);
       const float* cd = CDOF + k * NR;
 #pragma unroll
       for (int t = 0; t < 6; t++) s += cd[t] * V[t];
@@ -2651,7 +2682,7 @@
   }
   if constexpr (S::CL > 0) {
     const int f = lane >= 6 + S::CL ? 1 : 0, idx = lane - (6 + S::CL) * f;
-    const int c0 = f ? m->foot_rchain_first[1] : m->foot_rchain_first[0], cl = f ? m->foot_rchain_len[1] : m->foot_rchain_len[0];
+    const int c0 = f ? ODK_HOTI(HOT_RCHAIN_FIRST1, m->foot_rchain_first[1]) : ODK_HOTI(HOT_RCHAIN_FIRST0, m->foot_rchain_first[0]), cl = f ? ODK_HOTI(HOT_RCHAIN_LEN1, m->foot_rchain_len[1]) : ODK_HOTI(HOT_RCHAIN_LEN0, m->foot_rchain_len[0]);
     const bool lane_on = lane < 2 * (6 + S::CL) && idx - 6 < cl;
     const int col = lane_on ? (idx < 6 ? idx : c0 + idx - 6) : 0;
     const bool on = lane_on && ((f ? c_act[1] : c_act[0]) || c_act[2]);
@@ -2855,7 +2886,7 @@
       }
     }
   }
-  const float gtol = m->tolerance * m->ls_tolerance * sqrtf(sn) * m->meaninertia * (float)(NV > 1 ? NV : 1);
+  const float gtol = ODK_HOTF(HOT_F_TOL, m->tolerance) * ODK_HOTF(HOT_F_LSTOL, m->ls_tolerance) * sqrtf(sn) * ODK_HOTF(HOT_F_MEANI, m->meaninertia) * (float)(NV > 1 ? NV : 1);
   auto ls_eval = [&](auto cost_tag, const float* al, float* cost, float* d0, float* d1) {
     constexpr bool COST = decltype(cost_tag)::value;
     float acc[9] = {0, 0, 0, 0, 0, 0, 0, 0, 0};
@@ -2948,7 +2979,7 @@
   if (e0[0] < p0_d0) { lo_a = al[0]; lo_d0 = e0[0]; lo_d1 = e1[0]; hi_a = 0; hi_d0 = p0_d0; hi_d1 = p0_d1; }
   else { hi_a = al[0]; hi_d0 = e0[0]; hi_d1 = e1[0]; lo_a = 0; lo_d0 = p0_d0; lo_d1 = p0_d1; }
   bool swap = true;
-  for (int it = 0; it < m->ls_iterations; it++) {
+  for (int it = 0; it < ODK_HOTI(HOT_LS_ITERATIONS, m->ls_iterations); it++) {
     bool done = !swap || (lo_d0 < 0 && lo_d0 > -gtol) || (hi_d0 > 0 && hi_d0 < gtol);
     if (done) break;
     al[0] = lo_a - sdiv(lo_d0, lo_d1); al[1] = hi_a - sdiv(hi_d0, hi_d1); al[2] = 0.5f * (lo_a + hi_a);
diff --git a/open_duck_playground_amd/csrc/odk_model.h b/open_duck_playground_amd/csrc/odk_model.h
--- a/open_duck_playground_amd/csrc/odk_model.h
+++ b/open_duck_playground_amd/csrc/odk_model.h
@@ -23,6 +23,8 @@
 constexpr int MAXSENS = 16;
 constexpr int NCON = 12;
 constexpr int NSENSD = 46;
+constexpr int HOT_NPK = 3, HOT_NF = 17;
+constexpr int HOT_F_OBBC = 0, HOT_F_SPHR = 6, HOT_F_PLN = 8, HOT_F_PLP = 11, HOT_F_TOL = 14, HOT_F_LSTOL = 15, HOT_F_MEANI = 16;
 
 struct BodySt {
   int level, parent, child[4], njnt, jd[2], jj[2], jr[2], pathmask, is_path, upmask, path_head;
@@ -128,7 +130,19 @@
   int neq, eq_dof1[EQ_MAX], eq_dof2[EQ_MAX], eq_qadr1[EQ_MAX], eq_qadr2[EQ_MAX], eq_key[EQ_MAX], dof_eqrow[MAXV];
   float eq_poly[EQ_MAX][5], eq_imp[EQ_MAX][9], eq_invweight[EQ_MAX];
   alignas(16) ObsEnt obs_tab[2][OBS_MAX];
+  int hot_pk[HOT_NPK];
+  int np_rec[64][2];
+  float hot_f[HOT_NF];
 };
+struct HotField { const char* name; int word, shift, bits, scale; };
+constexpr HotField HOT_FOOT_BODY0 = {"foot_body[0]", 0, 0, 8, 4}, HOT_FOOT_BODY1 = {"foot_body[1]", 0, 8, 8, 4};
+constexpr HotField HOT_FOOT_NVERT0 = {"foot_nvert[0]", 0, 16, 8, 1}, HOT_FOOT_NVERT1 = {"foot_nvert[1]", 0, 24, 8, 1};
+constexpr HotField HOT_RCHAIN_FIRST0 = {"foot_rchain_first[0]", 1, 0, 8, 4}, HOT_RCHAIN_FIRST1 = {"foot_rchain_first[1]", 1, 8, 8, 4};
+constexpr HotField HOT_RCHAIN_LEN0 = {"foot_rchain_len[0]", 1, 16, 4, 1}, HOT_RCHAIN_LEN1 = {"foot_rchain_len[1]", 1, 20, 4, 1};
+constexpr HotField HOT_LS_ITERATIONS = {"ls_iterations", 1, 24, 8, 1};
+constexpr HotField HOT_NP_LEVELS = {"max_nonpath_level + 1", 2, 0, 8, 1}, HOT_NP_COUNT = {"np_count", 2, 8, 8, 1}, HOT_FOOT_PRIM = {"foot_prim", 2, 16, 8, 1};
+constexpr unsigned hot_stored(const int* pk, const HotField& f) { return ((unsigned)pk[f.word] >> f.shift) & ((1u << f.bits) - 1u); }
+constexpr int hot_value(const int* pk, const HotField& f) { return (int)(hot_stored(pk, f) / (unsigned)f.scale); }
 
 constexpr int PRISM_EDGE[9][4] = {{0, 1, 0, 2}, {1, 2, 0, 3}, {3, 5, 1, 4}, {0, 3, 2, 4}, {3, 4, 2, 1}, {1, 4, 3, 2}, {4, 5, 3, 1}, {2, 5, 4, 3}, {0, 2, 4, 0}};
 constexpr int PRISM_POLY[5][5] = {{3, 0, 1, 2, 0}, {3, 3, 5, 4, 3}, {4, 0, 3, 4, 1}, {4, 1, 4, 5, 2}, {4, 2, 5, 3, 0}};
diff --git a/open_duck_playground_amd/csrc/odk_model_load.hip b/open_duck_playground_amd/csrc/odk_model_load.hip
--- a/open_duck_playground_amd/csrc/odk_model_load.hip
+++ b/open_duck_playground_amd/csrc/odk_model_load.hip
@@ -906,6 +906,49 @@
 #undef X
   return 0;
 }
+
+int pack_hot(Load& c) {
+  DevModel& m = c.m;
+  const struct { const HotField& f; int v; } fields[] = {
+      {HOT_FOOT_BODY0, m.foot_body[0]},         {HOT_FOOT_BODY1, m.foot_body[1]},         {HOT_FOOT_NVERT0, m.foot_nvert[0]},     {HOT_FOOT_NVERT1, m.foot_nvert[1]},
+      {HOT_RCHAIN_FIRST0, m.foot_rchain_first[0]}, {HOT_RCHAIN_FIRST1, m.foot_rchain_first[1]}, {HOT_RCHAIN_LEN0, m.foot_rchain_len[0]}, {HOT_RCHAIN_LEN1, m.foot_rchain_len[1]},
+      {HOT_LS_ITERATIONS, m.ls_iterations},     {HOT_NP_LEVELS, m.max_nonpath_level + 1}, {HOT_NP_COUNT, m.np_count},             {HOT_FOOT_PRIM, m.foot_prim}};
+  for (int k = 0; k < HOT_NPK; k++) m.hot_pk[k] = 0;
+  for (const auto& e : fields) {
+    const long long stored = (long long)e.v * e.f.scale;
+    if (e.v < 0 || stored >= (1ll << e.f.bits))
+      return fail(ODK_ERR_UNSUPPORTED, "%s = %d does not fit the %d-bit field the step kernels read it from (0 .. %d)", e.f.name, e.v, e.f.bits,
+                  (int)(((1ll << e.f.bits) - 1) / e.f.scale));
+    m.hot_pk[e.f.word] |= (int)((unsigned)stored << e.f.shift);
+  }
+  for (int lane = 0; lane < 64; lane++) {
+    const int i = lane >> 4;
+    unsigned r0 = 0, r1 = 0;
+    if (i < m.np_count) {
+      const int* s = m.np_src[i];
+      r0 = (unsigned)(s[0] * 4) | (unsigned)(s[1] * 4) << 8 | (unsigned)(s[2] * 4) << 16 | (unsigned)(s[3] * 4) << 24;
+      r1 = (unsigned)(s[4] * 4) | (unsigned)(s[5] * 4) << 8 | (unsigned)(m.np_body[i] * 4) << 16 | (unsigned)m.np_nsrc[i] << 24;
+    }
+    m.np_rec[lane][0] = (int)r0; m.np_rec[lane][1] = (int)r1;
+  }
+  for (int f = 0; f < 2; f++) {
+    for (int k = 0; k < 3; k++) m.hot_f[HOT_F_OBBC + 3 * f + k] = m.foot_obb_center[f][k];
+    m.hot_f[HOT_F_SPHR + f] = m.foot_sphere_r[f];
+  }
+  for (int k = 0; k < 3; k++) { m.hot_f[HOT_F_PLN + k] = m.plane_n[k]; m.hot_f[HOT_F_PLP + k] = m.plane_pos[k]; }
+  m.hot_f[HOT_F_TOL] = m.tolerance; m.hot_f[HOT_F_LSTOL] = m.ls_tolerance; m.hot_f[HOT_F_MEANI] = m.meaninertia;
+  return 0;
+}
+}
+
+extern "C" int odk_model_hot_words(const odk_model* m, int* packed, int* fields) {
+  if (!m || !packed || !fields) return fail(ODK_ERR_INVALID, "odk_model_hot_words: bad arguments");
+  const DevModel& h = m->h;
+  for (int k = 0; k < HOT_NPK; k++) packed[k] = h.hot_pk[k];
+  const int v[12] = {h.foot_body[0], h.foot_body[1], h.foot_nvert[0], h.foot_nvert[1], h.foot_rchain_first[0], h.foot_rchain_first[1], h.foot_rchain_len[0], h.foot_rchain_len[1],
+                     h.ls_iterations, h.max_nonpath_level, h.np_count, h.foot_prim};
+  for (int k = 0; k < 12; k++) fields[k] = v[k];
+  return ODK_OK;
 }
 
 extern "C" int odk_model_load(const void* blob, uint64_t len, odk_model** out) {
@@ -916,7 +959,8 @@
   memset(&mo->h, 0, sizeof(mo->h));
   Load c{B, *mo, mo->h};
   int (*const stages[])(Load&) = {load_options, collect_equalities, load_tree,        load_actuators, load_rows,       load_feet,
-                                  load_floor,   load_sensors,       build_fold_lists, select_shape,   load_equalities, build_statics};
+                                  load_floor,   load_sensors,       build_fold_lists, select_shape,   load_equalities, build_statics,
+                                  pack_hot};
   for (auto stage : stages)
     if (const int err = stage(c)) return err;
   *out = mo.release();
diff --git a/open_duck_playground_amd/engine.py b/open_duck_playground_amd/engine.py
--- a/open_duck_playground_amd/engine.py
+++ b/open_duck_playground_amd/engine.py
@@ -396,6 +396,25 @@
         L.odk_model_free(h)
 
 
+HOT_FIELD_NAMES = ("foot_body0", "foot_body1", "foot_nvert0", "foot_nvert1", "foot_rchain_first0", "foot_rchain_first1", "foot_rchain_len0", "foot_rchain_len1",
+                   "ls_iterations", "max_nonpath_level", "np_count", "foot_prim")
+
+
+def model_hot_words(model: Model) -> Dict:
+    L = load_library()
+    L.odk_model_hot_words.argtypes = [C.c_void_p, C.POINTER(C.c_int), C.POINTER(C.c_int)]
+    L.odk_model_hot_words.restype = C.c_int
+    blob = model.blob()
+    h = C.c_void_p()
+    _chk(L.odk_model_load(blob, len(blob), C.byref(h)))
+    try:
+        packed, fields = (C.c_int * 3)(), (C.c_int * 12)()
+        _chk(L.odk_model_hot_words(h, packed, fields))
+        return dict(packed=[v & 0xFFFFFFFF for v in packed], fields=dict(zip(HOT_FIELD_NAMES, list(fields))))
+    finally:
+        L.odk_model_free(h)
+
+
 def model_body_lanes(model: Model, lanes_per_env: int) -> List[int]:
     L = load_library()
     blob = model.blob()
```

Measured after the change: 20.98 million (median of 6 runs). +1.8%, better.
